# hbaatz/nerf-tex

Hardware: AMD Instinct MI355X
Metric: ray-samples/sec (MLP+composite) at 800x800x64 (higher is better)
Workload: dtype f32; 1 GPU; carpet 800x800x64: 640000 all-hit rays x 64 samples per GPU (BASELINE configs[1]), ParamNerf n_parameters=[1, 6], seeded glorot weights, inputs resident in HBM, fused PE+MLP+composite; rays_per_gpu=640000, hit_rays_total=640000, samples_per_ray=64

## Files before the change

### nerf_tex_amd/csrc/ntx_train.hip

```cpp
#include "nerftex.h"

#include <hip/hip_runtime.h>

#include <algorithm>
#include <cmath>
#include <cstdint>
#include <cstdio>
#include <cstdlib>
#include <cstring>
#include <type_traits>
#include <vector>

#include "ntx_train_device.h"

extern "C" int ntx_set_error(int code, const char *fmt, ...);

#define TRAIN_TRY(expr)                                                                                  \
    do {                                                                                                 \
        hipError_t e_ = (expr);                                                                          \
        if (e_ != hipSuccess) return ntx_set_error(NTX_E_HIP, "%s: %s", #expr, hipGetErrorString(e_)); \
    } while (0)

namespace ntx_train {

constexpr int TM = 128;

struct GemmArgs {
    const float *A; int lda; const float *B; int ldb; float *C; int ldc;
    int M, N, K;
    const float *bias;
    const float *mask; int ldmask;
    int relu, accumulate;
    int k_chunk; long long split_stride;
    float *colsum;
    int aligned;
};

template <int n, bool FAST>
__device__ __forceinline__ void fetch_run(const float *g, bool row_ok, int first, int bound, float *r, bool aligned_ok = false) {
    if (FAST) {
        const f32x4 *v = reinterpret_cast<const f32x4 *>(g);
#pragma unroll
        for (int q = 0; q < n / 4; ++q) { const f32x4 x = v[q]; r[4 * q] = x.x; r[4 * q + 1] = x.y; r[4 * q + 2] = x.z; r[4 * q + 3] = x.w; }
    } else if (row_ok && first + n <= bound && aligned_ok) {
        const f32x4 *v = reinterpret_cast<const f32x4 *>(g);
#pragma unroll
        for (int q = 0; q < n / 4; ++q) { const f32x4 x = v[q]; r[4 * q] = x.x; r[4 * q + 1] = x.y; r[4 * q + 2] = x.z; r[4 * q + 3] = x.w; }
    } else {
#pragma unroll
        for (int q = 0; q < n; ++q) r[q] = (row_ok && first + q < bound) ? g[q] : 0.0f;
    }
}

template <bool A_KCONTIG, int TN_, int TK_>
__device__ __forceinline__ void gemm_body(const GemmArgs &g, int bx, int by, int bz) {
    constexpr int THREADS = TN_ * 2, WCOLS = TN_ / 64, LROWA = TM + 4, LROWB_ = TN_ + 4;
    constexpr int FA = TM * TK_ / THREADS;
    constexpr int FB = TN_ * TK_ / THREADS;
    constexpr int TPR = THREADS / TK_;
    static_assert(FA % 4 == 0 && FB % 4 == 0 && FA * (THREADS / TM) == TK_ && TPR * FB == TN_ && TPR * FA == TM, "panel split");
    __shared__ __attribute__((aligned(16))) float As[2][TK_][LROWA], Bs[2][TK_][LROWB_];
    const int lane = threadIdx.x & 63, wave = threadIdx.x >> 6;
    const int j0 = bx * TN_, i0 = by * TM;
    const int k_begin = bz * g.k_chunk;
    const int k_end = k_begin + g.k_chunk < g.K ? k_begin + g.k_chunk : g.K;
    float *C = g.C + (size_t)bz * (size_t)g.split_stride;
    f32x16 acc[2][2];
#pragma unroll
    for (int a = 0; a < 2; ++a)
#pragma unroll
        for (int b = 0; b < 2; ++b)
#pragma unroll
            for (int r = 0; r < 16; ++r) acc[a][b][r] = 0.0f;
    float ra[2][FA], rb[2][FB], cs[FB];
#pragma unroll
    for (int q = 0; q < FB; ++q) cs[q] = 0.0f;
    const bool want_colsum = !A_KCONTIG && g.colsum != nullptr && by == 0;
    const bool inner = g.aligned && i0 + TM <= g.M && j0 + TN_ <= g.N;
    const int a_row = A_KCONTIG ? (int)(threadIdx.x % TM) : (int)(threadIdx.x / TPR), a_off = A_KCONTIG ? (int)(threadIdx.x / TM) * FA : (int)(threadIdx.x % TPR) * FA;
    const int b_row = (int)(threadIdx.x / TPR), b_off = (int)(threadIdx.x % TPR) * FB;
    auto fetch = [&](int k0, float *fa, float *fb) {
        const bool al = g.aligned != 0;
        if (A_KCONTIG) fetch_run<FA, false>(g.A + (size_t)(i0 + a_row) * g.lda + k0 + a_off, i0 + a_row < g.M, k0 + a_off, k_end, fa, al);
        else fetch_run<FA, false>(g.A + (size_t)(k0 + a_row) * g.lda + i0 + a_off, k0 + a_row < k_end, i0 + a_off, g.M, fa, al);
        fetch_run<FB, false>(g.B + (size_t)(k0 + b_row) * g.ldb + j0 + b_off, k0 + b_row < k_end, j0 + b_off, g.N, fb, al);
    };
    auto stash = [&](int buf, const float *fa, const float *fb) {
        if (want_colsum) {
#pragma unroll
            for (int q = 0; q < FB; ++q) cs[q] += fb[q];
        }
        if (A_KCONTIG) {
#pragma unroll
            for (int q = 0; q < FA; ++q) As[buf][a_off + q][a_row] = fa[q];
        } else {
            f32x4 *d = reinterpret_cast<f32x4 *>(&As[buf][a_row][a_off]);
#pragma unroll
            for (int q = 0; q < FA / 4; ++q) d[q] = f32x4{fa[4 * q], fa[4 * q + 1], fa[4 * q + 2], fa[4 * q + 3]};
        }
        f32x4 *d = reinterpret_cast<f32x4 *>(&Bs[buf][b_row][b_off]);
#pragma unroll
        for (int q = 0; q < FB / 4; ++q) d[q] = f32x4{fb[4 * q], fb[4 * q + 1], fb[4 * q + 2], fb[4 * q + 3]};
    };
    const int n_panels = (k_end - k_begin + TK_ - 1) / TK_;
    const int n_full = inner ? (k_end - k_begin) / TK_ : 0;
    const int wi = (wave / WCOLS) * 64 + 2 * (lane & 31), wj = (wave % WCOLS) * 64 + 2 * (lane & 31), kh = lane >> 5;
    const bool wave_live = j0 + (wave % WCOLS) * 64 < g.N;
    auto compute = [&](int buf) {
        if (!wave_live) return;
        f32x2 av[2], bv[2];
        av[0] = *reinterpret_cast<const f32x2 *>(&As[buf][kh][wi]); bv[0] = *reinterpret_cast<const f32x2 *>(&Bs[buf][kh][wj]);
#pragma unroll
        for (int st = 0; st < TK_ / 2; ++st) {
            const int c = st & 1, n = c ^ 1;
            if (st + 1 < TK_ / 2) {
                const int kk = 2 * (st + 1) + kh;
                av[n] = *reinterpret_cast<const f32x2 *>(&As[buf][kk][wi]); bv[n] = *reinterpret_cast<const f32x2 *>(&Bs[buf][kk][wj]);
            }
            __builtin_amdgcn_sched_barrier(0);
            acc[0][0] = __builtin_amdgcn_mfma_f32_32x32x2f32(av[c].x, bv[c].x, acc[0][0], 0, 0, 0);
            acc[0][1] = __builtin_amdgcn_mfma_f32_32x32x2f32(av[c].x, bv[c].y, acc[0][1], 0, 0, 0);
            acc[1][0] = __builtin_amdgcn_mfma_f32_32x32x2f32(av[c].y, bv[c].x, acc[1][0], 0, 0, 0);
            acc[1][1] = __builtin_amdgcn_mfma_f32_32x32x2f32(av[c].y, bv[c].y, acc[1][1], 0, 0, 0);
            __builtin_amdgcn_sched_barrier(0);
        }
    };
    auto fetch_fast = [&](int k0, float *fa, float *fb) {
        const float *ga = A_KCONTIG ? g.A + (size_t)(i0 + a_row) * g.lda + k0 + a_off : g.A + (size_t)(k0 + a_row) * g.lda + i0 + a_off;
        fetch_run<FA, true>(ga, true, 0, 0, fa);
        fetch_run<FB, true>(g.B + (size_t)(k0 + b_row) * g.ldb + j0 + b_off, true, 0, 0, fb);
    };
    auto pipeline = [&](auto fast_tag, int first, int last) {
        constexpr bool FAST = decltype(fast_tag)::value;
        auto get = [&](int kt, float *fa, float *fb) { if (FAST) fetch_fast(k_begin + kt * TK_, fa, fb); else fetch(k_begin + kt * TK_, fa, fb); };
        if (first >= last) return;
        get(first, ra[0], rb[0]); stash(0, ra[0], rb[0]);
        if (first + 1 < last) get(first + 1, ra[1], rb[1]);
        __syncthreads();
        int kt = first;
        for (; kt + 3 < last; kt += 2) {
            get(kt + 2, ra[0], rb[0]); compute(0); stash(1, ra[1], rb[1]); __syncthreads();
            get(kt + 3, ra[1], rb[1]); compute(1); stash(0, ra[0], rb[0]); __syncthreads();
        }
        for (; kt < last; ++kt) {
            const int buf = (kt - first) & 1;
            if (kt + 2 < last) { if (buf) get(kt + 2, ra[1], rb[1]); else get(kt + 2, ra[0], rb[0]); }
            compute(buf);
            if (kt + 1 < last) { if (buf) stash(0, ra[0], rb[0]); else stash(1, ra[1], rb[1]); }
            __syncthreads();
        }
    };
    pipeline(std::true_type{}, 0, n_full);
    pipeline(std::false_type{}, n_full, n_panels);
    const bool whole = i0 + TM <= g.M && j0 + TN_ <= g.N && (g.ldc % 2 == 0) && (!g.mask || g.ldmask % 2 == 0) && ((uintptr_t)C % 8 == 0) && ((uintptr_t)g.mask % 8 == 0);
    const int j = j0 + (wave % WCOLS) * 64 + 2 * (lane & 31);
    const float bj0 = (g.bias && j < g.N) ? g.bias[j] : 0.0f, bj1 = (g.bias && j + 1 < g.N) ? g.bias[j + 1] : 0.0f;
#pragma unroll
    for (int a = 0; a < 2; ++a)
#pragma unroll
        for (int r = 0; r < 16; ++r) {
            const int i = i0 + (wave / WCOLS) * 64 + 2 * (8 * (r >> 2) + (r & 3) + 4 * kh) + a;
            float v0 = acc[a][0][r], v1 = acc[a][1][r];
            float *c = C + (size_t)i * g.ldc + j;
            if (whole) {
                f32x2 *c2 = reinterpret_cast<f32x2 *>(c);
                if (g.accumulate) { const f32x2 o = *c2; v0 += o.x; v1 += o.y; }
                v0 += bj0; v1 += bj1;
                if (g.relu) { v0 = v0 > 0.0f ? v0 : 0.0f; v1 = v1 > 0.0f ? v1 : 0.0f; }
                if (g.mask) { const f32x2 mk = *reinterpret_cast<const f32x2 *>(g.mask + (size_t)i * g.ldmask + j); if (!(mk.x > 0.0f)) v0 = 0.0f; if (!(mk.y > 0.0f)) v1 = 0.0f; }
                *c2 = f32x2{v0, v1};
            } else if (i < g.M) {
#pragma unroll
                for (int b = 0; b < 2; ++b) {
                    if (j + b >= g.N) continue;
                    float v = b ? v1 : v0;
                    if (g.accumulate) v = v + c[b];
                    v = v + (b ? bj1 : bj0);
                    if (g.relu) v = v > 0.0f ? v : 0.0f;
                    if (g.mask && !(g.mask[(size_t)i * g.ldmask + j + b] > 0.0f)) v = 0.0f;
                    c[b] = v;
                }
            }
        }
    if (want_colsum) {
        float (*red)[LROWB_] = Bs[0];
#pragma unroll
        for (int q = 0; q < FB; ++q) red[b_row][b_off + q] = cs[q];
        __syncthreads();
        if ((int)threadIdx.x < TN_ && j0 + (int)threadIdx.x < g.N) {
            float sum = 0.0f;
            for (int q = 0; q < TK_; ++q) sum += red[q][threadIdx.x];
            g.colsum[(size_t)bz * g.N + j0 + threadIdx.x] = sum;
        }
    }
}


__device__ __forceinline__ void gemm_place(int lin, int nx, int ny, int nz, int &bx, int &by, int &bz) {
    const int tiles = nx * ny;
    if (nz % 8 == 0) {
        const int xcd = lin & 7, slot = lin >> 3, tile = slot % tiles;
        bz = (slot / tiles) * 8 + xcd; bx = tile % nx; by = tile / nx;
    } else { bx = lin % nx; by = (lin / nx) % ny; bz = lin / tiles; }
}
template <bool A_KCONTIG, int TN_, int TK_, int WAVES_PER_EU = 2>
__global__ __launch_bounds__(TN_ * 2) __attribute__((amdgpu_waves_per_eu(WAVES_PER_EU, 8))) void gemm_kernel(GemmArgs g) {
    int bx, by, bz;
    gemm_place(blockIdx.x + gridDim.x * (blockIdx.y + gridDim.y * blockIdx.z), gridDim.x, gridDim.y, gridDim.z, bx, by, bz);
    gemm_body<A_KCONTIG, TN_, TK_>(g, bx, by, bz);
}

constexpr int MAX_REDUCE_BATCH = 32;
struct ReduceJob { const float *partial; int n_split; long long stride, count, pair; float *out; long long first; };
struct ReduceBatch { ReduceJob job[MAX_REDUCE_BATCH]; int n; };
__global__ void reduce_batch_kernel(ReduceBatch b) {
    const long long g = (long long)blockIdx.x * blockDim.x + threadIdx.x;
    int j = 0;
    while (j + 1 < b.n && g >= b.job[j + 1].first) ++j;
    const ReduceJob &r = b.job[j];
    const long long e = g - r.first;
    if (e >= r.count) return;
    float s4[4] = {0.0f, 0.0f, 0.0f, 0.0f};
    auto at = [&](int z) { const float *p = r.partial + (size_t)z * r.stride + e; return r.pair > 0 ? p[0] + p[r.pair] : p[0]; };
    int z = 0;
    for (; z + 4 <= r.n_split; z += 4) {
#pragma unroll
        for (int q = 0; q < 4; ++q) s4[q] += at(z + q);
    }
    for (int q = 0; z < r.n_split; ++z, ++q) s4[q] += at(z);
    r.out[e] = (s4[0] + s4[1]) + (s4[2] + s4[3]);
}

enum { PACK_HIDDEN = 0, PACK_LINEAR = 1, PACK_AUX_ROW = 2, PACK_AUX_RGB = 3, PACK_COPY = 4 };
struct PackSeg {
    const float *src; long long sk, sc;
    int mode;
    int K, ncols, nt;
    float *dst; long long first, count;
};
struct PackArgs { const PackSeg *seg; int n_seg; long long total; };
__global__ void pack_kernel(PackArgs a) {
    const long long e = (long long)blockIdx.x * blockDim.x + threadIdx.x;
    if (e >= a.total) return;
    int lo = 0, hi = a.n_seg - 1;
    while (lo < hi) { const int mid = (lo + hi + 1) >> 1; if (a.seg[mid].first <= e) lo = mid; else hi = mid - 1; }
    const PackSeg &p = a.seg[lo];
    const long long o = e - p.first;
    float v = 0.0f;
    if (p.mode == PACK_COPY) v = p.src[o];
    else if (p.mode == PACK_AUX_ROW) {
        const int h = (int)(o >> 7) & 1, V = (int)(o & 127), k = hidden_row(V, h);
        v = k < p.K ? p.src[k * p.sk] : 0.0f;
    } else if (p.mode == PACK_AUX_RGB) {
        const int c = (int)(o >> 7), h = (int)(o >> 6) & 1, V = (int)(o & 63);
        v = p.src[hidden_row(V, h) * 3 + c];
    } else {
        const int c = (int)(o & 3), lane = (int)((o >> 2) & 63);
        const long long rec = o >> 8;
        const int G = p.nt / 4, g = (int)(rec % G), s = (int)(rec / G);
        const int f = lane & 31, kh = lane >> 5;
        const int k = p.mode == PACK_HIDDEN ? hidden_row(s, kh) : 2 * s + kh, col = 32 * (4 * g + c) + f;
        if (k < p.K && col < p.ncols) v = p.src[k * p.sk + col * p.sc];
    }
    p.dst[o] = v;
}

struct EncodeArgs {
    const float *rays_o, *rays_d, *z, *params, *cone;
    long long rays_per_param_row, M;
    int n_rays, S, n_geo, n_app, pos_freq, dir_freq, param_freq, blur_idx;
    float *posO; int ptiles;
    float *dirO; int dtiles;
    float *dists;
};
__global__ __launch_bounds__(64) void encode_kernel(EncodeArgs a) {
    const int lane = threadIdx.x, n = lane & 31, h = lane >> 5, blk = blockIdx.x, part = blockIdx.y;
    const long long m = (long long)blk * 32 + n;
    const bool valid = m < a.M;
    const int ray = valid ? (int)(m / a.S) : 0, s = valid ? (int)(m - (long long)ray * a.S) : 0;
    const float d[3] = {a.rays_d[3 * ray], a.rays_d[3 * ray + 1], a.rays_d[3 * ray + 2]};
    const float dn = sqrtf((d[0] * d[0] + d[1] * d[1]) + d[2] * d[2]);
    const float zr = a.z[(size_t)ray * a.S + s];
    const bool hit = isfinite(zr);
    const float z = hit ? zr : 0.0f;
    const int P = a.n_geo + a.n_app;
    const float *pr = a.params + (size_t)(ray / a.rays_per_param_row) * (P > 0 ? P : 1);
    auto param = [&](int c) { return c == a.blur_idx ? (hit ? pr[c] * (a.cone[ray] * z) : 0.0f) : pr[c]; };
    float *O = part == 0 ? a.posO : a.dirO;
    const int tiles = part == 0 ? a.ptiles : a.dtiles;
    auto put = [&](int row, float v) {
        if (!valid) v = 0.0f;
        O[(((size_t)blk * tiles + (row >> 5)) * 4 + (n >> 3)) * 256 + ((row & 31) + 32 * ((n >> 2) & 1)) * 4 + (n & 3)] = v;
    };
    auto fourier = [&](int r0, int D, int L, auto x) {
        if (h == 0) for (int c = 0; c < D; ++c) put(r0 + c, x(c));
        for (int f = 0; f < L; ++f)
            for (int c = 0; c < D; ++c) put(r0 + D + 2 * D * f + h * D + c, ntx::sin_q(ldexpf(1.0f, f) * x(c), h));
    };
    if (part == 0) {
        const float o[3] = {a.rays_o[3 * ray], a.rays_o[3 * ray + 1], a.rays_o[3 * ray + 2]};
        fourier(0, 3, a.pos_freq, [&](int c) { return o[c] + d[c] * z; });
        if (a.n_geo > 0) fourier(3 * (1 + 2 * a.pos_freq), a.n_geo, a.param_freq, [&](int c) { return param(c); });
    } else {
        fourier(0, 3, a.dir_freq, [&](int c) { return d[c] / dn; });
        if (a.n_app > 0) fourier(3 * (1 + 2 * a.dir_freq), a.n_app, a.param_freq, [&](int c) { return param(a.n_geo + c); });
        if (valid && h == 0) {
            const float zn = s + 1 < a.S ? a.z[(size_t)ray * a.S + s + 1] : 0.0f;
            const float dist = s + 1 < a.S ? zn - z : (a.S > 1 ? z - a.z[(size_t)ray * a.S + s - 1] : 0.0f);
            a.dists[(size_t)ray * a.S + s] = hit ? dist * dn : 0.0f;
        }
    }
}

__global__ __launch_bounds__(64) void encode_ipe_kernel(EncodeArgs a) {
    const int lane = threadIdx.x, n = lane & 31, h = lane >> 5, blk = blockIdx.x, part = blockIdx.y;
    const long long m = (long long)blk * 32 + n;
    const bool valid = m < a.M;
    const int ray = valid ? (int)(m / a.S) : 0, s = valid ? (int)(m - (long long)ray * a.S) : 0;
    const float d[3] = {a.rays_d[3 * ray], a.rays_d[3 * ray + 1], a.rays_d[3 * ray + 2]};
    const float dn = sqrtf((d[0] * d[0] + d[1] * d[1]) + d[2] * d[2]);
    const float *zr = a.z + (size_t)ray * (a.S + 1) + s;
    const float e0 = zr[0], e1 = zr[1];
    const bool hit = isfinite(e0) && isfinite(e1);
    const int P = a.n_geo + a.n_app;
    const float *pr = a.params + (size_t)(ray / a.rays_per_param_row) * (P + 1);
    auto param = [&](int k) { return pr[k < a.blur_idx ? k : k + 1]; };
    float *O = part == 0 ? a.posO : a.dirO;
    const int tiles = part == 0 ? a.ptiles : a.dtiles;
    auto put = [&](int row, float v) {
        if (!valid) v = 0.0f;
        O[(((size_t)blk * tiles + (row >> 5)) * 4 + (n >> 3)) * 256 + ((row & 31) + 32 * ((n >> 2) & 1)) * 4 + (n & 3)] = v;
    };
    auto fourier = [&](int r0, int D, int L, auto x) {
        if (h == 0) for (int c = 0; c < D; ++c) put(r0 + c, x(c));
        for (int f = 0; f < L; ++f)
            for (int c = 0; c < D; ++c) put(r0 + D + 2 * D * f + h * D + c, ntx::sin_q(ldexpf(1.0f, f) * x(c), h));
    };
    if (part == 0) {
        float mean[3] = {a.rays_o[3 * ray], a.rays_o[3 * ray + 1], a.rays_o[3 * ray + 2]}, cov[3] = {0.0f, 0.0f, 0.0f};
        if (hit) {
            float t_mean, t_var, r_var;
            ntx::cone_moments((e0 + e1) / 2.0f, (e1 - e0) / 2.0f, pr[a.blur_idx] * a.cone[ray], t_mean, t_var, r_var);
            for (int c = 0; c < 3; ++c) mean[c] = mean[c] + d[c] * t_mean;
            ntx::cone_cov(t_var, r_var, d, cov);
        }
        const int L = a.pos_freq;
        for (int f = 0; f < L; ++f)
            for (int c = 0; c < 3; ++c)
                put(h * 3 * L + 3 * f + c, ntx::sin_q(mean[c] * ldexpf(1.0f, f), h) * expf(-0.5f * (cov[c] * ldexpf(1.0f, 2 * f))));
        if (a.n_geo > 0) fourier(6 * L, a.n_geo, a.param_freq, [&](int c) { return param(c); });
    } else {
        fourier(0, 3, a.dir_freq, [&](int c) { return d[c] / dn; });
        if (a.n_app > 0) fourier(3 * (1 + 2 * a.dir_freq), a.n_app, a.param_freq, [&](int c) { return param(a.n_geo + c); });
        if (valid && h == 0) a.dists[(size_t)ray * a.S + s] = hit ? (e1 - e0) * dn : 0.0f;
    }
}

struct DirRowArgs {
    const float *rays_d, *params; long long rays_per_param_row;
    int n_rays, n_geo, n_app, dir_freq, param_freq, Kd, splice;
    const float *w, *bias;
    float *rows;
};
__global__ __launch_bounds__(256) void dirrow_kernel(DirRowArgs a) {
    __shared__ float feat[8 * MAX_PB_GROUPS];
    const int ray = blockIdx.x, f = threadIdx.x;
    const float d[3] = {a.rays_d[3 * ray], a.rays_d[3 * ray + 1], a.rays_d[3 * ray + 2]};
    const float dn = sqrtf((d[0] * d[0] + d[1] * d[1]) + d[2] * d[2]);
    const int P = a.n_geo + a.n_app + (a.splice >= 0 ? 1 : 0);
    const float *pr = a.params + (size_t)(ray / a.rays_per_param_row) * (P > 0 ? P : 1);
    if (f < a.Kd) {
        const int K3 = 3 * (1 + 2 * a.dir_freq);
        const int r = f < K3 ? f : f - K3, D = f < K3 ? 3 : a.n_app;
        auto x = [&](int c) { const int k = a.n_geo + c; return f < K3 ? d[c] / dn : pr[a.splice >= 0 && k >= a.splice ? k + 1 : k]; };
        float v;
        if (r < D) v = x(r);
        else { const int q = r - D, band = q / (2 * D), hc = q - band * 2 * D, hh = hc / D, c = hc - hh * D; v = ntx::sin_q(ldexpf(1.0f, band) * x(c), hh); }
        feat[f] = v;
    }
    __syncthreads();
    float acc = a.bias[f];
    for (int k = 0; k < a.Kd; ++k) acc = fmaf(feat[k], a.w[(size_t)k * 256 + f], acc);
    const int T = f >> 5, g = (f >> 3) & 3, h = (f >> 2) & 1, c = f & 3;
    a.rows[(size_t)ray * 256 + h * 128 + 16 * T + 4 * g + c] = acc;
}

struct CompositeArgs {
    const float *raw_rgb, *sigma, *dists;
    const float *noise;
    int n_rays, S, map_exr, composite_bkgd; float bkgd[3];
    const float *color_true, *alpha_true;
    int kind, loss_fn, alpha_loss_fn, filter_color_loss, use_hard_mask; float gamma;
    float *color, *alpha, *ray_loss;
    float *weights;
    float *dgrad;
    float *dhead;
    long long M;
};
constexpr int MAX_TRAIN_SAMPLES = 1024;
__device__ __forceinline__ float wave_sumf(float v) { for (int o = 32; o > 0; o >>= 1) v += __shfl_xor(v, o); return v; }
__device__ __forceinline__ float rgb_of(float raw, int map_exr) {
    if (map_exr) return raw > 0.0f ? raw + 1.0f : expf(raw);
    return 1.0f / (1.0f + expf(-raw));
}
__device__ __forceinline__ void loss_term(int fn, float t, float p, float inv_n, float &value, float &grad) {
    if (fn == NTX_LOSS_MSE) { const float e = t - p; value = e * e * inv_n; grad = -2.0f * e * inv_n; }
    else {
        const float e = t - p, den = (t + p) + 1e-2f, ae = fabsf(e);
        const float sgn = e > 0.0f ? 1.0f : (e < 0.0f ? -1.0f : 0.0f);
        value = ae / den * inv_n; grad = (-sgn / den - ae / (den * den)) * inv_n;
    }
}
__device__ __forceinline__ size_t dhead_at(long long m, int row) {
    const long long blk = m >> 5; const int p = (int)(m & 31);
    return (size_t)((blk * 4 + (p >> 3)) * 256 + (row + 32 * ((p >> 2) & 1)) * 4 + (p & 3));
}
__global__ __launch_bounds__(256) void composite_loss_kernel(CompositeArgs a) {
    __shared__ float sh_a[4][MAX_TRAIN_SAMPLES], sh_T[4][MAX_TRAIN_SAMPLES];
    const int lane = threadIdx.x & 63, wave = threadIdx.x >> 6;
    if (blockIdx.x == 0) {
        const long long end = (a.M + 31) / 32 * 32;
        for (long long m = a.M + threadIdx.x; m < end; m += 256)
            for (int r = 0; r < 4; ++r) a.dhead[dhead_at(m, r)] = 0.0f;
    }
    const int ray = blockIdx.x * 4 + wave;
    if (ray >= a.n_rays) return;
    const int S = a.S;
    const float *sg = a.sigma + (size_t)ray * S, *ds = a.dists + (size_t)ray * S, *rr = a.raw_rgb + (size_t)ray * S * 3;
    const float *nz = a.noise ? a.noise + (size_t)ray * S : nullptr;
    float *el = sh_a[wave], *T = sh_T[wave];
    for (int s = lane; s < S; s += 64) { const float v = nz ? sg[s] + nz[s] : sg[s]; const float r = v > 0.0f ? v : 0.0f; el[s] = expf(-r * ds[s]); }
    __builtin_amdgcn_wave_barrier();
    float carry = 1.0f;
    for (int s0 = 0; s0 < S; s0 += 64) {
        const int s = s0 + lane;
        float f = s < S ? el[s] + 1e-10f : 1.0f, incl = f;
        for (int o = 1; o < 64; o <<= 1) { const float w = __shfl_up(incl, o); if (lane >= o) incl *= w; }
        float excl = __shfl_up(incl, 1);
        if (lane == 0) excl = 1.0f;
        if (s < S) T[s] = carry * excl;
        carry *= __shfl(incl, 63);
    }
    __builtin_amdgcn_wave_barrier();
    float c0 = 0.0f, c1 = 0.0f, c2 = 0.0f, A = 0.0f;
    for (int s = lane; s < S; s += 64) {
        const float w = (1.0f - el[s]) * T[s];
        c0 += w * rgb_of(rr[3 * s], a.map_exr); c1 += w * rgb_of(rr[3 * s + 1], a.map_exr); c2 += w * rgb_of(rr[3 * s + 2], a.map_exr);
        A += w;
        if (a.weights) a.weights[(size_t)ray * S + s] = w;
    }
    c0 = wave_sumf(c0); c1 = wave_sumf(c1); c2 = wave_sumf(c2); A = wave_sumf(A);
    if (a.composite_bkgd) { c0 += (1.0f - A) * a.bkgd[0]; c1 += (1.0f - A) * a.bkgd[1]; c2 += (1.0f - A) * a.bkgd[2]; }
    const float cp[3] = {c0, c1, c2};
    float dC[3], dA = 0.0f, total = 0.0f;
    {
        const float inv_c = 1.0f / (float)(a.n_rays * 3), inv_a = 1.0f / (float)a.n_rays;
        float mask = 1.0f;
        if (a.kind == NTX_LOSS_ALPHA && a.filter_color_loss) mask = a.use_hard_mask ? (a.alpha_true[ray] > 0.0f ? 1.0f : 0.0f) : a.alpha_true[ray];
        for (int c = 0; c < 3; ++c) {
            float v, gr;
            loss_term(a.loss_fn, a.color_true[3 * ray + c] * mask, cp[c] * mask, inv_c, v, gr);
            total += v; dC[c] = gr * mask;
        }
        if (a.kind == NTX_LOSS_ALPHA) { float v; loss_term(a.alpha_loss_fn, a.alpha_true[ray], A, inv_a, v, dA); total += a.gamma * v; dA *= a.gamma; }
    }
    if (lane == 0) { a.color[3 * ray] = c0; a.color[3 * ray + 1] = c1; a.color[3 * ray + 2] = c2; a.alpha[ray] = A; a.ray_loss[ray] = total; }
    if (a.composite_bkgd) dA -= (dC[0] * a.bkgd[0] + dC[1] * a.bkgd[1]) + dC[2] * a.bkgd[2];
    float Z_carry = 1.0f, V_carry = 0.0f;
    for (int s0 = ((S - 1) / 64) * 64; s0 >= 0; s0 -= 64) {
        const int s = s0 + lane;
        float cs = 0.0f, rgb[3] = {0.0f, 0.0f, 0.0f}, e = 1.0f;
        float F = 1.0f, Bz = 0.0f, Bv = 0.0f;
        if (s < S) {
            e = el[s];
            for (int c = 0; c < 3; ++c) rgb[c] = rgb_of(rr[3 * s + c], a.map_exr);
            cs = (dC[0] * rgb[0] + dC[1] * rgb[1]) + dC[2] * rgb[2];
            F = e + 1e-10f; Bz = -1e-10f; Bv = cs * (1.0f - e);
        }
        for (int o = 1; o < 64; o <<= 1) {
            const float Fo = __shfl_down(F, o), Bzo = __shfl_down(Bz, o), Bvo = __shfl_down(Bv, o);
            if (lane + o < 64) { Bz = fmaf(F, Bzo, Bz); Bv = fmaf(F, Bvo, Bv); F *= Fo; }
        }
        float Fn = __shfl_down(F, 1), Bzn = __shfl_down(Bz, 1), Bvn = __shfl_down(Bv, 1);
        if (lane == 63) { Fn = 1.0f; Bzn = 0.0f; Bvn = 0.0f; }
        const float Z = fmaf(Fn, Z_carry, Bzn), V = fmaf(Fn, V_carry, Bvn);
        if (s < S) {
            const float w = (1.0f - e) * T[s];
            const float d_a = T[s] * fmaf(dA, Z, cs - V);
            const float sig = nz ? sg[s] + nz[s] : sg[s];
            float gr[4];
            for (int c = 0; c < 3; ++c) {
                const float raw = rr[3 * s + c];
                const float drgb = a.map_exr ? (raw > 0.0f ? 1.0f : expf(raw)) : rgb[c] * (1.0f - rgb[c]);
                gr[c] = w * dC[c] * drgb;
            }
            gr[3] = sig > 0.0f ? d_a * ds[s] * e : 0.0f;
            const long long m = (long long)ray * S + s;
            *reinterpret_cast<f32x4 *>(a.dgrad + 4 * m) = f32x4{gr[0], gr[1], gr[2], gr[3]};
            for (int r = 0; r < 4; ++r) a.dhead[dhead_at(m, r)] = gr[r];
        }
        const float F0 = __shfl(F, 0);
        Z_carry = fmaf(F0, Z_carry, __shfl(Bz, 0)); V_carry = fmaf(F0, V_carry, __shfl(Bv, 0));
    }
}
__global__ __launch_bounds__(1024) void loss_sum_kernel(const float *__restrict__ ray_loss, int n_rays, float *__restrict__ loss) {
    __shared__ float red[1024];
    float total = 0.0f;
    for (int r = threadIdx.x; r < n_rays; r += blockDim.x) total += ray_loss[r];
    red[threadIdx.x] = total;
    __syncthreads();
    for (int o = blockDim.x / 2; o > 0; o >>= 1) { if ((int)threadIdx.x < o) red[threadIdx.x] += red[threadIdx.x + o]; __syncthreads(); }
    if (threadIdx.x == 0) *loss = red[0];
}

__global__ void adam_kernel(float *__restrict__ w, const float *__restrict__ g, float *__restrict__ m, float *__restrict__ v, long long n, float lr_t, float b1,
                            float b2, float eps) {
    const long long e = (long long)blockIdx.x * blockDim.x + threadIdx.x;
    if (e >= n) return;
    const float ge = g[e];
    const float me = m[e] + (ge - m[e]) * (1.0f - b1);
    const float ve = v[e] + (ge * ge - v[e]) * (1.0f - b2);
    m[e] = me; v[e] = ve;
    w[e] = w[e] - (me * lr_t) / (sqrtf(ve) + eps);
}

}

struct TLayer { int in, out; size_t w, b; };

struct ntx_trainer {
    int device = 0, cus = 256;
    ntx_model_desc desc{};
    int Kp = 0, Kd = 0, P = 0, ptiles = 0, dtiles = 0, PS = 0, DS = 0;
    bool ipe = false;
    TLayer trunk[8], feature, c1, c2, rgb, alpha;
    size_t n_weights = 0;
    long long cap = 0, cap_blocks = 0, cap_rays = 0;
    float *w = nullptr, *grad = nullptr, *adam_m = nullptr, *adam_v = nullptr;
    float *wfwd = nullptr, *wdx = nullptr, *aux = nullptr; size_t fwd_floats = 0, dx_floats = 0;
    ntx_train::PackSeg *pack_seg = nullptr; int n_pack = 0; long long pack_total = 0;
    float *posO = nullptr, *dirO = nullptr;
    float *act = nullptr; long long act_stride = 0;
    unsigned int *bits = nullptr; long long bits_stride = 0;
    int fwd_variant = 0;
    float *sigma = nullptr, *raw_rgb = nullptr, *z = nullptr, *dists = nullptr, *noise = nullptr;
    float *dirrow = nullptr;
    float *dgrad = nullptr, *dhead = nullptr, *gout = nullptr; long long gout_stride = 0;
    ntx_train::DwJob *jobs = nullptr; int n_jobs = 0; long long total_cost = 0;
    std::vector<ntx_train::DwJob> jobs_host; std::vector<int> reduce_job;
    float *dw_partial = nullptr;
    ntx_train::ReduceBatch reduce{};
    float *color = nullptr, *alpha_out = nullptr, *ray_loss = nullptr, *loss = nullptr;
    float *weights_out = nullptr;
    float *stash = nullptr;
    long long adam_iterations = 0;
};

namespace {

using namespace ntx_train;


void free_all(ntx_trainer *t) {
    if (!t) return;
    (void)hipSetDevice(t->device);
    void *ptrs[] = {t->w, t->grad, t->adam_m, t->adam_v, t->wfwd, t->wdx, t->aux, t->pack_seg, t->posO, t->dirO, t->sigma, t->raw_rgb, t->z, t->dists, t->noise,
                    t->dgrad, t->dhead, t->jobs, t->dw_partial, t->stash, t->dirrow, t->color, t->alpha_out, t->ray_loss, t->loss, t->act, t->bits, t->gout};
    for (void *p : ptrs) if (p) (void)hipFree(p);
    delete t;
}

template <bool AK>
void launch_gemm(hipStream_t st, GemmArgs g) {
    g.k_chunk = g.K;
    g.aligned = (g.lda % 4 == 0) && (g.ldb % 4 == 0) && (((uintptr_t)g.A | (uintptr_t)g.B) % 16 == 0);
    hipLaunchKernelGGL((gemm_kernel<AK, 128, 16>), dim3((g.N + 127) / 128, (g.M + TM - 1) / TM, 1), dim3(256), 0, st, g);
}

}

namespace ntx_train {
template <int K, bool HOIST> void launch_fwd_variant(hipStream_t st, unsigned grid, const FwdArgs &a);
void launch_fwd_chain(int variant, bool hoist, hipStream_t st, unsigned grid, const FwdArgs &a) {
    switch (variant * 2 + (hoist ? 1 : 0)) {
        case 0: launch_fwd_variant<0, false>(st, grid, a); break;
        case 1: launch_fwd_variant<0, true>(st, grid, a); break;
        case 2: launch_fwd_variant<1, false>(st, grid, a); break;
        case 3: launch_fwd_variant<1, true>(st, grid, a); break;
        case 4: launch_fwd_variant<2, false>(st, grid, a); break;
        case 5: launch_fwd_variant<2, true>(st, grid, a); break;
        case 6: launch_fwd_variant<3, false>(st, grid, a); break;
        default: launch_fwd_variant<3, true>(st, grid, a); break;
    }
}
}

extern "C" {

int ntx_sample_depths(const float *t, int64_t n_rays, int n_points, uint32_t flags, uint64_t perturb_seed, const ntx_render_opts *opts, float *z_out,
                      ntx_stream stream);
int ntx_sample_noise(int64_t n_rays, int n_points, uint64_t seed, const ntx_render_opts *opts, float *noise_out, ntx_stream stream);

int ntx_trainer_create(const ntx_model_desc *desc, const float *weights, size_t n_floats, int device, int64_t max_rays, int max_samples_per_ray, ntx_trainer **out) {
    if (!out) return ntx_set_error(NTX_E_INVALID, "out is NULL");
    *out = nullptr;
    if (!desc || !weights) return ntx_set_error(NTX_E_INVALID, "desc / weights is NULL");
    const bool ipe = desc->pos_encoding == NTX_POS_IPE && desc->n_pos == 6;
    if (desc->kind != NTX_MODEL_PARAMNERF || desc->depth != 8 || desc->width != 256 || desc->skip != 4 || desc->color_depth != 1 ||
        !((desc->pos_encoding == NTX_POS_FOURIER && desc->n_pos == 3) || ipe))
        return ntx_set_error(NTX_E_UNSUPPORTED, "training is built for the ParamNerf architecture of the shipped training configs (depth 8, width 256, skips [4], color_depth 1, "
                                                "Fourier features on n_pos 3 or IPE on n_pos 6); others render but do not train");
    if (desc->n_geo < 0 || desc->n_app < 0 || desc->n_geo + desc->n_app > 16) return ntx_set_error(NTX_E_INVALID, "n_parameters out of range");
    if (desc->pos_freq < 0 || desc->dir_freq < 0 || desc->param_freq < 0) return ntx_set_error(NTX_E_INVALID, "negative band count");
    const int Kp = (ipe ? 6 * desc->pos_freq : 3 * (1 + 2 * desc->pos_freq)) + desc->n_geo * (1 + 2 * desc->param_freq), Kd = 3 * (1 + 2 * desc->dir_freq) + desc->n_app * (1 + 2 * desc->param_freq);
    if (Kp > 8 * MAX_PB_GROUPS || Kd > 8 * MAX_PB_GROUPS)
        return ntx_set_error(NTX_E_UNSUPPORTED, "training: pos_map (%d) / dir_map (%d) wider than %d features (the chain holds a block's encoded inputs in registers)", Kp, Kd,
                             8 * MAX_PB_GROUPS);
    if (max_rays < 1 || max_samples_per_ray < 2 || max_samples_per_ray > MAX_TRAIN_SAMPLES || max_rays * (int64_t)max_samples_per_ray > (int64_t)1 << 30)
        return ntx_set_error(NTX_E_INVALID, "max_rays / max_samples_per_ray out of range (samples per ray <= %d)", MAX_TRAIN_SAMPLES);
    int ndev = 0;
    if (hipGetDeviceCount(&ndev) != hipSuccess || ndev <= 0) return ntx_set_error(NTX_E_NODEVICE, "no HIP device visible");
    if (device < 0 || device >= ndev) return ntx_set_error(NTX_E_INVALID, "device %d out of range [0,%d)", device, ndev);
    ntx_trainer *t = new ntx_trainer();
    t->device = device; t->desc = *desc; t->ipe = ipe;
    t->P = desc->n_geo + desc->n_app; t->Kp = Kp; t->Kd = Kd;
    t->ptiles = (Kp + 31) / 32; t->dtiles = (Kd + 31) / 32;
    {
        const int psg = ((Kp + 1) / 2 + 3) / 4, dsg = ((Kd + 1) / 2 + 3) / 4;
        t->fwd_variant = 3;
        for (int v = 2; v >= 0; --v)
            if (FWD_VARIANTS[v][0] >= psg && FWD_VARIANTS[v][1] >= dsg &&
                FWD_VARIANTS[v][0] + FWD_VARIANTS[v][1] <= FWD_VARIANTS[t->fwd_variant][0] + FWD_VARIANTS[t->fwd_variant][1]) t->fwd_variant = v;
        t->PS = 4 * FWD_VARIANTS[t->fwd_variant][0]; t->DS = 4 * FWD_VARIANTS[t->fwd_variant][1];
    }
    size_t p = 0;
    auto take = [&](int in, int o) { TLayer l{in, o, p, p + (size_t)in * o}; p += (size_t)in * o + o; return l; };
    int k = Kp;
    for (int i = 0; i < 8; ++i) { t->trunk[i] = take(k, 256); k = 256 + (i == 4 ? Kp : 0); }
    t->feature = take(256, 256); t->c1 = take(256 + Kd, 256); t->c2 = take(256, 128); t->rgb = take(128, 3); t->alpha = take(256, 1);
    t->n_weights = p;
    if (n_floats != p) { delete t; return ntx_set_error(NTX_E_INVALID, "weights: %zu floats, the model has %zu", n_floats, p); }
    const long long M = (long long)max_rays * max_samples_per_ray, NB = (M + 31) / 32;
    t->cap = M; t->cap_rays = max_rays; t->cap_blocks = NB;
    int rc = hipSetDevice(device) == hipSuccess ? NTX_OK : ntx_set_error(NTX_E_HIP, "hipSetDevice(%d) failed", device);
    if (rc == NTX_OK) { int n = 0; if (hipDeviceGetAttribute(&n, hipDeviceAttributeMultiprocessorCount, device) == hipSuccess && n > 0) t->cus = n; }
    auto alloc = [&](float **d, size_t n, bool zero = false) -> int {
        if (rc != NTX_OK) return rc;
        if (hipMalloc((void **)d, (n ? n : 1) * sizeof(float)) != hipSuccess) return rc = ntx_set_error(NTX_E_HIP, "hipMalloc of %zu floats failed", n);
        if (zero && hipMemset(*d, 0, (n ? n : 1) * sizeof(float)) != hipSuccess) return rc = ntx_set_error(NTX_E_HIP, "hipMemset failed");
        return rc;
    };
    alloc(&t->w, p); alloc(&t->grad, p, true); alloc(&t->adam_m, p, true); alloc(&t->adam_v, p, true);
    alloc(&t->posO, (size_t)NB * t->ptiles * 1024, true); alloc(&t->dirO, (size_t)NB * t->dtiles * 1024, true);
    t->act_stride = t->gout_stride = NB * 8 * 1024; t->bits_stride = NB * 256;
    alloc(&t->act, (size_t)t->act_stride * 11); alloc((float **)&t->bits, (size_t)t->bits_stride * 10); alloc(&t->gout, (size_t)t->gout_stride * 11);
    auto act = [&](int i) { return t->act + (size_t)i * t->act_stride; };
    auto gout = [&](int i) { return t->gout + (size_t)i * t->gout_stride; };
    alloc(&t->sigma, (size_t)M); alloc(&t->raw_rgb, (size_t)M * 3); alloc(&t->z, (size_t)(M + max_rays)); alloc(&t->dists, (size_t)M); alloc(&t->noise, (size_t)M);
    alloc(&t->dirrow, (size_t)max_rays * 256);
    alloc(&t->dgrad, (size_t)NB * 32 * 4); alloc(&t->dhead, (size_t)NB * 1024, true);
    alloc(&t->color, (size_t)max_rays * 3); alloc(&t->alpha_out, (size_t)max_rays); alloc(&t->ray_loss, (size_t)max_rays); alloc(&t->loss, 1);
    if (rc == NTX_OK && hipMemcpy(t->w, weights, p * sizeof(float), hipMemcpyHostToDevice) != hipSuccess) rc = ntx_set_error(NTX_E_HIP, "weight upload failed");
    std::vector<PackSeg> segs;
    long long first = 0;
    auto seg = [&](const float *src, long long sk, long long sc, int mode, int K, int ncols, int nt, size_t *stream_floats, int nsteps) {
        PackSeg s{}; s.src = src; s.sk = sk; s.sc = sc; s.mode = mode; s.K = K; s.ncols = ncols; s.nt = nt;
        const int ring = stream_floats == &t->dx_floats ? DX_RING : RING;
        const long long recs = ((long long)nsteps * (nt / 4) + ring - 1) / ring * ring;
        s.count = recs * 256; s.first = first; s.dst = (float *)(uintptr_t)(*stream_floats * sizeof(float));
        first += s.count; *stream_floats += (size_t)s.count;
        segs.push_back(s);
    };
    const float *W = t->w;
    auto fwd_hidden = [&](const TLayer &l, int row0, int nt) { seg(W + l.w + (size_t)row0 * l.out, l.out, 1, PACK_HIDDEN, 256, l.out, nt, &t->fwd_floats, 128); };
    auto fwd_linear = [&](const TLayer &l, int K, int nsteps) { seg(W + l.w, l.out, 1, PACK_LINEAR, K, l.out, 8, &t->fwd_floats, nsteps); };
    fwd_linear(t->trunk[0], Kp, t->PS);
    for (int i = 1; i < 8; ++i) {
        if (i == 5) { fwd_linear(t->trunk[5], Kp, t->PS); fwd_hidden(t->trunk[5], Kp, 8); }
        else fwd_hidden(t->trunk[i], 0, 8);
    }
    fwd_hidden(t->feature, 0, 8);
    fwd_linear(t->c1, Kd, t->DS); fwd_hidden(t->c1, Kd, 8);
    fwd_hidden(t->c2, 0, 4);
    const size_t n_fwd_segs = segs.size();
    auto dx_hidden = [&](const TLayer &l, int row0, int K, int nsteps) { seg(W + l.w + (size_t)row0 * l.out, 1, l.out, PACK_HIDDEN, K, 256, 8, &t->dx_floats, nsteps); };
    seg(W + t->rgb.w, 1, 3, PACK_LINEAR, 3, 128, 4, &t->dx_floats, 2);
    dx_hidden(t->c2, 0, 128, 64);
    dx_hidden(t->c1, Kd, 256, 128);
    dx_hidden(t->feature, 0, 256, 128);
    seg(W + t->alpha.w, 1, 1, PACK_LINEAR, 1, 256, 8, &t->dx_floats, 1);
    for (int i = 7; i >= 1; --i) dx_hidden(t->trunk[i], i == 5 ? Kp : 0, 256, 128);
    const size_t n_stream_segs = segs.size();
    auto tail = [&](size_t of, size_t *stream_floats) { PackSeg s = segs[of]; s.count = (long long)(stream_floats == &t->dx_floats ? DX_RING : RING) * 256; s.first = first; s.dst = (float *)(uintptr_t)(*stream_floats * sizeof(float));
                                                        first += s.count; *stream_floats += (size_t)s.count; segs.push_back(s); };
    tail(0, &t->fwd_floats); tail(n_fwd_segs, &t->dx_floats);
    auto aux_seg = [&](const float *src, int mode, int K, long long count, size_t at) {
        PackSeg s{}; s.src = src; s.sk = 1; s.mode = mode; s.K = K; s.count = count; s.first = first; s.dst = (float *)(uintptr_t)(at * sizeof(float));
        first += count; segs.push_back(s);
    };
    for (int i = 0; i < 8; ++i) aux_seg(W + t->trunk[i].b, PACK_AUX_ROW, 256, 256, AUX_BIAS + (size_t)i * 256);
    aux_seg(W + t->feature.b, PACK_AUX_ROW, 256, 256, AUX_BIAS + 8 * 256); aux_seg(W + t->c1.b, PACK_AUX_ROW, 256, 256, AUX_BIAS + 9 * 256);
    aux_seg(W + t->c2.b, PACK_AUX_ROW, 128, 256, AUX_BIAS + 10 * 256);
    aux_seg(W + t->alpha.w, PACK_AUX_ROW, 256, 256, AUX_ALPHA_W); aux_seg(W + t->alpha.b, PACK_COPY, 1, 1, AUX_ALPHA_B);
    aux_seg(W + t->rgb.w, PACK_AUX_RGB, 128, 384, AUX_RGB_W); aux_seg(W + t->rgb.b, PACK_COPY, 3, 3, AUX_RGB_B);
    t->pack_total = first; t->n_pack = (int)segs.size();
    alloc(&t->wfwd, t->fwd_floats); alloc(&t->wdx, t->dx_floats); alloc(&t->aux, AUX_FLOATS, true);
    if (rc == NTX_OK) {
        for (size_t i = 0; i < segs.size(); ++i) {
            const bool is_aux = i >= n_stream_segs + 2, is_fwd = i < n_fwd_segs || i == n_stream_segs;
            float *base = is_aux ? t->aux : is_fwd ? t->wfwd : t->wdx;
            segs[i].dst = (float *)((char *)base + (uintptr_t)segs[i].dst);
        }
        if (hipMalloc((void **)&t->pack_seg, segs.size() * sizeof(PackSeg)) != hipSuccess ||
            hipMemcpy(t->pack_seg, segs.data(), segs.size() * sizeof(PackSeg), hipMemcpyHostToDevice) != hipSuccess)
            rc = ntx_set_error(NTX_E_HIP, "segment table upload failed");
    }
    std::vector<DwJob> &jobs = t->jobs_host;
    struct RJ { int job; long long at, count, pair; size_t out; };
    std::vector<RJ> rjobs;
    auto new_job = [&]() { DwJob j{}; for (DwWave &w : j.w) w.shape = -1; jobs.push_back(j); return (int)jobs.size() - 1; };
    auto matrix = [&](int j, int K, int N, size_t g_kernel, long long g_bias, long long *at_bias) {
        const long long at = jobs[j].slot_floats;
        jobs[j].slot_floats += (long long)K * N;
        rjobs.push_back(RJ{j, at, (long long)K * N, 0, g_kernel});
        *at_bias = -1;
        if (g_bias >= 0) { *at_bias = jobs[j].slot_floats; jobs[j].slot_floats += 2 * N; rjobs.push_back(RJ{j, *at_bias, N, N, (size_t)g_bias}); }
        return at;
    };
    auto wave = [&](int j, int w, int shape, const float *A, int rtA, int a0, const float *B, int rtB, int b0, long long at, int K, int N, int c_lo, long long at_bias) {
        DwWave &d = jobs[j].w[w];
        d.A = A; d.rtA = rtA; d.a0 = a0; d.B = B; d.rtB = rtB; d.b0 = b0; d.shape = shape; d.out = at; d.ldc = N; d.row0 = a0 * 32; d.rows_valid = K;
        d.col0 = b0 * 32; d.c_lo = c_lo; d.c_hi = c_lo + N; d.bias_out = a0 == 0 ? at_bias : -1;
        const int cost = shape == 0 ? 256 : shape == 1 ? 198 : 68;
        if (cost > jobs[j].cost) jobs[j].cost = cost;
    };
    auto layer_job = [&](const float *X, const float *dY, size_t g_kernel, size_t g_bias) {
        const int j = new_job(); long long ab; const long long at = matrix(j, 256, 256, g_kernel, (long long)g_bias, &ab);
        for (int w = 0; w < 4; ++w) wave(j, w, 0, X, 8, 4 * (w >> 1), dY, 8, 4 * (w & 1), at, 256, 256, 0, ab);
    };
    {
        const TLayer &r = t->rgb, &al = t->alpha, &c2 = t->c2, &c1 = t->c1, &f = t->feature;
        for (int i = 7; i >= 1; --i) layer_job(act(i - 1), gout(10 - i), t->trunk[i].w + (size_t)(i == 5 ? Kp : 0) * 256, t->trunk[i].b);
        layer_job(act(7), gout(2), f.w, f.b);
        layer_job(act(8), gout(1), c1.w + (size_t)Kd * 256, c1.b);
        {
            const int j = new_job(); long long ab0, ab5;
            const long long at0 = matrix(j, Kp, 256, t->trunk[0].w, (long long)t->trunk[0].b, &ab0), at5 = matrix(j, Kp, 256, t->trunk[5].w, -1, &ab5);
            for (int w = 0; w < 2; ++w) { wave(j, w, 1, t->posO, t->ptiles, 0, gout(10), 8, 4 * w, at0, Kp, 256, 0, ab0); wave(j, 2 + w, 1, t->posO, t->ptiles, 0, gout(5), 8, 4 * w, at5, Kp, 256, 0, ab5); }
        }
        {
            const int j = new_job(); long long abd, ab2;
            const long long atd = matrix(j, Kd, 256, c1.w, -1, &abd), at2 = matrix(j, 256, 128, c2.w, (long long)c2.b, &ab2);
            for (int w = 0; w < 2; ++w) { wave(j, w, 1, t->dirO, t->dtiles, 0, gout(1), 8, 4 * w, atd, Kd, 256, 0, abd); wave(j, 2 + w, 0, act(9), 8, 4 * w, gout(0), 4, 0, at2, 256, 128, 0, ab2); }
        }
        {
            const int j = new_job(); long long abr, aba;
            const long long atr = matrix(j, 128, 3, r.w, (long long)r.b, &abr), ata = matrix(j, 256, 1, al.w, (long long)al.b, &aba);
            wave(j, 0, 2, act(10), 4, 0, t->dhead, 1, 0, atr, 128, 3, 0, abr);
            for (int w = 0; w < 2; ++w) wave(j, 1 + w, 2, act(7), 8, 4 * w, t->dhead, 1, 0, ata, 256, 1, 3, aba);
        }
    }
    t->n_jobs = (int)jobs.size();
    size_t partial_floats = 0;
    for (DwJob &j : jobs) {
        t->total_cost += j.cost;
    }
    for (DwJob &j : jobs) {
        const long long slots = ((long long)j.cost * t->cus + t->total_cost - 1) / t->total_cost + 2;
        j.first_float = (long long)partial_floats; partial_floats += (size_t)(slots * j.slot_floats);
    }
    alloc(&t->dw_partial, partial_floats);
    if (rc == NTX_OK) {
        if (hipMalloc((void **)&t->jobs, jobs.size() * sizeof(DwJob)) != hipSuccess ||
            hipMemcpy(t->jobs, jobs.data(), jobs.size() * sizeof(DwJob), hipMemcpyHostToDevice) != hipSuccess)
            rc = ntx_set_error(NTX_E_HIP, "job table upload failed");
        if ((int)rjobs.size() > MAX_REDUCE_BATCH) rc = ntx_set_error(NTX_E_INVALID, "trainer: too many weight gradients for one launch");
        long long rfirst = 0;
        for (size_t i = 0; i < rjobs.size() && rc == NTX_OK; ++i) {
            ReduceJob &r = t->reduce.job[t->reduce.n++];
            const DwJob &j = jobs[rjobs[i].job];
            r.partial = t->dw_partial + j.first_float + rjobs[i].at; r.n_split = 0; r.stride = j.slot_floats; r.count = rjobs[i].count; r.pair = rjobs[i].pair;
            r.out = t->grad + rjobs[i].out; r.first = rfirst;
            rfirst += (rjobs[i].count + 255) / 256 * 256;
            t->reduce_job.push_back(rjobs[i].job);
        }
    }
    if (rc != NTX_OK) { free_all(t); return rc; }
    *out = t;
    return NTX_OK;
}

int ntx_trainer_destroy(ntx_trainer *t) { free_all(t); return NTX_OK; }

size_t ntx_trainer_weight_count(const ntx_trainer *t) { return t ? t->n_weights : 0; }

static float *trainer_vector(ntx_trainer *t, int what) {
    return what == NTX_TRAINER_WEIGHTS ? t->w : what == NTX_TRAINER_GRADIENTS ? t->grad : what == NTX_TRAINER_ADAM_M ? t->adam_m : what == NTX_TRAINER_ADAM_V ? t->adam_v : nullptr;
}

int ntx_trainer_get(ntx_trainer *t, int what, float *out_host, size_t n_floats) {
    if (!t || !out_host) return ntx_set_error(NTX_E_INVALID, "NULL argument");
    if (n_floats != t->n_weights) return ntx_set_error(NTX_E_INVALID, "%zu floats asked, the model has %zu", n_floats, t->n_weights);
    const float *src = trainer_vector(t, what);
    if (!src) return ntx_set_error(NTX_E_INVALID, "what = %d", what);
    TRAIN_TRY(hipSetDevice(t->device));
    TRAIN_TRY(hipDeviceSynchronize());
    TRAIN_TRY(hipMemcpy(out_host, src, n_floats * sizeof(float), hipMemcpyDeviceToHost));
    return NTX_OK;
}

int ntx_trainer_activation(ntx_trainer *t, int layer, int64_t n_samples_total, float *out_host) {
    if (!t || !out_host) return ntx_set_error(NTX_E_INVALID, "NULL argument");
    if (n_samples_total < 1 || n_samples_total > t->cap) return ntx_set_error(NTX_E_INVALID, "n_samples_total out of range");
    const float *src = nullptr; int tiles = 8;
    auto act = [&](int i) { return t->act + (size_t)i * t->act_stride; };
    auto gout = [&](int i) { return t->gout + (size_t)i * t->gout_stride; };
    if (layer >= 0 && layer < 8) src = act(layer);
    else if (layer == 8) src = act(9);
    else if (layer == 9) { src = act(10); tiles = 4; }
    else if (layer == 10) src = t->sigma;
    else if (layer >= 20 && layer < 28) src = gout(10 - (layer - 20));
    else if (layer == 28) src = gout(1);
    else if (layer == 29) src = gout(2);
    else if (layer == 11) src = t->raw_rgb;
    else if (layer == 30) src = t->dgrad;
    else return ntx_set_error(NTX_E_INVALID, "layer %d (0-7 trunk, 8 / 9 the colour layers, 10 the density, 11 the raw colour; 20-29 the kept gradients, 30 the composite's adjoint)", layer);
    TRAIN_TRY(hipSetDevice(t->device));
    TRAIN_TRY(hipDeviceSynchronize());
    if (layer == 10 || layer == 11 || layer == 30) {
        const size_t width = layer == 10 ? 1 : (layer == 11 ? 3 : 4);
        TRAIN_TRY(hipMemcpy(out_host, src, (size_t)n_samples_total * width * sizeof(float), hipMemcpyDeviceToHost)); return NTX_OK;
    }
    const long long nb = (n_samples_total + 31) / 32;
    std::vector<float> tmp((size_t)nb * tiles * 1024);
    TRAIN_TRY(hipMemcpy(tmp.data(), src, tmp.size() * sizeof(float), hipMemcpyDeviceToHost));
    const int width = tiles * 32;
    for (long long m = 0; m < n_samples_total; ++m) {
        const long long blk = m >> 5; const int p = (int)(m & 31);
        const float *rec = tmp.data() + ((size_t)blk * tiles * 4 + (p >> 3)) * 256 + 32 * ((p >> 2) & 1) * 4 + (p & 3);
        float *o = out_host + (size_t)m * width;
        for (int T = 0; T < tiles; ++T)
            for (int i = 0; i < 32; ++i) o[32 * T + i] = rec[(size_t)T * 1024 + i * 4];
    }
    return NTX_OK;
}

int ntx_trainer_set_weights(ntx_trainer *t, const float *weights_host, size_t n_floats) { return ntx_trainer_set(t, NTX_TRAINER_WEIGHTS, weights_host, n_floats); }

int ntx_trainer_set(ntx_trainer *t, int what, const float *values_host, size_t n_floats) {
    if (!t || !values_host) return ntx_set_error(NTX_E_INVALID, "NULL argument");
    if (n_floats != t->n_weights) return ntx_set_error(NTX_E_INVALID, "%zu floats given, the model has %zu", n_floats, t->n_weights);
    float *dst = trainer_vector(t, what);
    if (!dst) return ntx_set_error(NTX_E_INVALID, "what = %d", what);
    TRAIN_TRY(hipSetDevice(t->device));
    TRAIN_TRY(hipDeviceSynchronize());
    TRAIN_TRY(hipMemcpy(dst, values_host, n_floats * sizeof(float), hipMemcpyHostToDevice));
    return NTX_OK;
}

int ntx_trainer_set_iterations(ntx_trainer *t, int64_t iterations) {
    if (!t || iterations < 0) return ntx_set_error(NTX_E_INVALID, "trainer is NULL or iterations < 0");
    t->adam_iterations = iterations;
    return NTX_OK;
}

int ntx_trainer_composite_weights(ntx_trainer *t, float *weights_dev) {
    if (!t) return ntx_set_error(NTX_E_INVALID, "trainer is NULL");
    if (t->ipe && weights_dev) return ntx_set_error(NTX_E_UNSUPPORTED, "an IPE trainer has no importance pass (MipRenderer: renderer.py:403-404)");
    t->weights_out = weights_dev;
    return NTX_OK;
}

namespace ntx_train {
__global__ void add_kernel(float *__restrict__ dst, const float *__restrict__ src, long long n) {
    const long long e = (long long)blockIdx.x * blockDim.x + threadIdx.x;
    if (e < n) dst[e] += src[e];
}
}

int ntx_trainer_stash_gradients(ntx_trainer *t, int op, ntx_stream stream) {
    if (!t || (op != 0 && op != 1)) return ntx_set_error(NTX_E_INVALID, "trainer is NULL or op is not 0 (keep) / 1 (add back)");
    TRAIN_TRY(hipSetDevice(t->device));
    if (!t->stash) {
        if (op == 1) return ntx_set_error(NTX_E_INVALID, "no gradient was kept");
        TRAIN_TRY(hipMalloc((void **)&t->stash, t->n_weights * sizeof(float)));
    }
    if (op == 0) TRAIN_TRY(hipMemcpyAsync(t->stash, t->grad, t->n_weights * sizeof(float), hipMemcpyDeviceToDevice, (hipStream_t)stream));
    else hipLaunchKernelGGL(ntx_train::add_kernel, dim3((unsigned)((t->n_weights + 255) / 256)), dim3(256), 0, (hipStream_t)stream, t->grad, t->stash, (long long)t->n_weights);
    TRAIN_TRY(hipGetLastError());
    return NTX_OK;
}

int ntx_trainer_device_weights(ntx_trainer *t, const float **weights_dev) {
    if (!t || !weights_dev) return ntx_set_error(NTX_E_INVALID, "NULL argument");
    *weights_dev = t->w;
    return NTX_OK;
}

int ntx_trainer_allreduce_gradients(ntx_trainer *t, ntx_comm *comm, ntx_stream stream) {
    if (!t || !comm) return ntx_set_error(NTX_E_INVALID, "NULL argument");
    return ntx_allreduce_mean_f32(comm, t->grad, t->n_weights, stream);
}

int ntx_train_step_gradients(ntx_trainer *t, const float *rays_o, const float *rays_d, const float *tnear_far, const float *params, int64_t rays_per_param_row,
                             const float *cone_scale, int64_t n_rays, int n_samples, int blur_idx, uint32_t flags, const float *bkgd, uint64_t perturb_seed,
                             const ntx_render_opts *opts, const float *z_vals, const float *color_true, const float *alpha_true, const ntx_loss_desc *loss,
                             float *color_pred, float *alpha_pred, float *loss_out, ntx_stream stream) {
    if (!t) return ntx_set_error(NTX_E_INVALID, "trainer is NULL");
    const int P_in = t->P + (t->ipe ? 1 : 0);
    if (!rays_o || !rays_d || (!tnear_far && !z_vals) || !color_true || !loss || (P_in > 0 && !params)) return ntx_set_error(NTX_E_INVALID, "NULL buffer");
    if (n_rays < 1 || n_rays > t->cap_rays || n_samples < 2 || (long long)n_rays * n_samples > t->cap) return ntx_set_error(NTX_E_INVALID, "n_rays x n_samples beyond what the trainer was created for");
    if (n_samples > MAX_TRAIN_SAMPLES) return ntx_set_error(NTX_E_INVALID, "n_samples > %d", MAX_TRAIN_SAMPLES);
    if (blur_idx >= P_in || (blur_idx >= 0 && !cone_scale) || (t->ipe && blur_idx < 0)) return ntx_set_error(NTX_E_INVALID, "bad blur_idx / cone_scale");
    if (loss->size < sizeof(ntx_loss_desc) || (loss->kind != NTX_LOSS_NERF && loss->kind != NTX_LOSS_ALPHA) || (loss->loss_fn != NTX_LOSS_MSE && loss->loss_fn != NTX_LOSS_SMAPE) ||
        (loss->alpha_loss_fn != NTX_LOSS_MSE && loss->alpha_loss_fn != NTX_LOSS_SMAPE))
        return ntx_set_error(NTX_E_INVALID, "bad ntx_loss_desc");
    if (loss->kind == NTX_LOSS_ALPHA && !alpha_true) return ntx_set_error(NTX_E_INVALID, "AlphaLoss needs alpha_true");
    if (rays_per_param_row < 1) rays_per_param_row = 1;
    TRAIN_TRY(hipSetDevice(t->device));
    hipStream_t st = (hipStream_t)stream;
    const long long M = (long long)n_rays * n_samples;
    const int S = n_samples, n_blocks = (int)((M + 31) / 32);
    {
        PackArgs pa{t->pack_seg, t->n_pack, t->pack_total};
        hipLaunchKernelGGL(pack_kernel, dim3((unsigned)((t->pack_total + 255) / 256)), dim3(256), 0, st, pa);
    }
    const float *z = z_vals;
    if (!z) {
        int rc = ntx_sample_depths(tnear_far, n_rays, t->ipe ? S + 1 : S, flags & NTX_FLAG_PERTURB, perturb_seed, opts, t->z, stream);
        if (rc != NTX_OK) return rc;
        z = t->z;
    }
    const float *noise = nullptr;
    if (flags & NTX_FLAG_RAW_NOISE) {
        int rc = ntx_sample_noise(n_rays, S, perturb_seed, opts, t->noise, stream);
        if (rc != NTX_OK) return rc;
        noise = t->noise;
    }
    {
        EncodeArgs e{}; e.rays_o = rays_o; e.rays_d = rays_d; e.z = z; e.params = params; e.cone = cone_scale; e.rays_per_param_row = rays_per_param_row; e.M = M;
        e.n_rays = (int)n_rays; e.S = S; e.n_geo = t->desc.n_geo; e.n_app = t->desc.n_app; e.pos_freq = t->desc.pos_freq; e.dir_freq = t->desc.dir_freq;
        e.param_freq = t->desc.param_freq; e.blur_idx = blur_idx; e.posO = t->posO; e.ptiles = t->ptiles; e.dirO = t->dirO;
        e.dtiles = t->dtiles; e.dists = t->dists;
        if (t->ipe) hipLaunchKernelGGL(encode_ipe_kernel, dim3((unsigned)n_blocks, 2), dim3(64), 0, st, e);
        else hipLaunchKernelGGL(encode_kernel, dim3((unsigned)n_blocks, 2), dim3(64), 0, st, e);
    }
    const unsigned chain_grid = (unsigned)std::min<long long>(t->cus, (n_blocks + 3) / 4);
    {
        FwdArgs f{}; f.stream = t->wfwd; f.stream_bytes = (uint32_t)(t->fwd_floats * sizeof(float)); f.aux = t->aux; f.M = M;
        f.ptiles = t->ptiles; f.dtiles = t->dtiles; f.pos = t->posO; f.dir = t->dirO;
        f.act = t->act; f.act_stride = t->act_stride; f.bits = t->bits; f.bits_stride = t->bits_stride;
        f.sigma = t->sigma; f.raw_rgb = t->raw_rgb;
        const bool hoist = (t->ipe || blur_idx < 0 || blur_idx < t->desc.n_geo) && S % 32 == 0 && getenv("NERFTEX_TRAIN_NO_DIR_HOIST") == nullptr;
        if (hoist) {
            DirRowArgs dr{}; dr.rays_d = rays_d; dr.params = params; dr.rays_per_param_row = rays_per_param_row; dr.n_rays = (int)n_rays; dr.n_geo = t->desc.n_geo;
            dr.n_app = t->desc.n_app; dr.dir_freq = t->desc.dir_freq; dr.param_freq = t->desc.param_freq; dr.Kd = t->Kd; dr.w = t->w + t->c1.w; dr.bias = t->w + t->c1.b;
            dr.rows = t->dirrow; dr.splice = t->ipe ? blur_idx : -1;
            hipLaunchKernelGGL(dirrow_kernel, dim3((unsigned)n_rays), dim3(256), 0, st, dr);
        }
        f.dirrow = t->dirrow; f.n_rays = (int)n_rays; f.S = S;
        launch_fwd_chain(t->fwd_variant, hoist, st, chain_grid, f);
    }
    {
        CompositeArgs c{};
        c.raw_rgb = t->raw_rgb; c.sigma = t->sigma; c.dists = t->dists; c.noise = noise; c.n_rays = (int)n_rays; c.S = S; c.map_exr = (flags & NTX_FLAG_MAP_EXR) ? 1 : 0;
        c.composite_bkgd = (flags & NTX_FLAG_COMPOSITE_BKGD) ? 1 : 0;
        for (int k = 0; k < 3; ++k) c.bkgd[k] = bkgd ? bkgd[k] : 1.0f;
        c.color_true = color_true; c.alpha_true = alpha_true; c.kind = loss->kind; c.loss_fn = loss->loss_fn; c.alpha_loss_fn = loss->alpha_loss_fn;
        c.filter_color_loss = loss->filter_color_loss; c.use_hard_mask = loss->use_hard_mask; c.gamma = loss->gamma;
        c.weights = t->weights_out;
        c.color = color_pred ? color_pred : t->color; c.alpha = alpha_pred ? alpha_pred : t->alpha_out; c.ray_loss = t->ray_loss; c.dgrad = t->dgrad; c.dhead = t->dhead; c.M = M;
        hipLaunchKernelGGL(composite_loss_kernel, dim3((unsigned)((n_rays + 3) / 4)), dim3(256), 0, st, c);
        hipLaunchKernelGGL(loss_sum_kernel, dim3(1), dim3(1024), 0, st, t->ray_loss, (int)n_rays, loss_out ? loss_out : t->loss);
    }
    {
        DxArgs d{}; d.stream = t->wdx; d.stream_bytes = (uint32_t)(t->dx_floats * sizeof(float)); d.M = M; d.dgrad = t->dgrad;
        d.out = t->gout; d.out_stride = t->gout_stride; d.bits = t->bits; d.bits_stride = t->bits_stride;
        launch_dx_chain(st, chain_grid, d);
    }
    {
        DwArgs d{}; d.jobs = t->jobs; d.n_jobs = t->n_jobs; d.n_blocks = n_blocks; d.total_cost = t->total_cost; d.partial = t->dw_partial;
        const long long G = t->cus, W = t->total_cost * n_blocks;
#ifdef NTX_TRAIN_CLOCKS
        static unsigned long long *clocks = nullptr;
        const size_t nck = (size_t)G * (2 + 3 * t->n_jobs);
        if (getenv("NERFTEX_DW_CLOCKS")) {
            if (!clocks) (void)hipMalloc((void **)&clocks, nck * sizeof(unsigned long long));
            (void)hipMemsetAsync(clocks, 0, nck * sizeof(unsigned long long), st);
            d.clocks = clocks;
        }
#endif
        launch_dw(st, (unsigned)G, d);
#ifdef NTX_TRAIN_CLOCKS
        if (d.clocks) {
            std::vector<unsigned long long> h(nck);
            (void)hipStreamSynchronize(st);
            (void)hipMemcpy(h.data(), clocks, nck * sizeof(unsigned long long), hipMemcpyDeviceToHost);
            unsigned long long t0 = ~0ull;
            for (long long g = 0; g < G; ++g) t0 = std::min(t0, h[g * (2 + 3 * t->n_jobs)]);
            FILE *f = fopen(getenv("NERFTEX_DW_CLOCKS"), "w");
            if (f) {
                for (long long g = 0; g < G; ++g) {
                    const unsigned long long *c = &h[g * (2 + 3 * t->n_jobs)];
                    fprintf(f, "%lld %llu %llu", g, c[0] - t0, c[1] - t0);
                    for (int j = 0; j < t->n_jobs; ++j) if (c[4 + 3 * j]) fprintf(f, "  j%d cost %d blocks %llu %llu-%llu", j, t->jobs_host[j].cost, c[2 + 3 * j], c[3 + 3 * j] - t0, c[4 + 3 * j] - t0);
                    fprintf(f, "\n");
                }
                fclose(f);
            }
        }
#endif
        ReduceBatch rb = t->reduce;
        std::vector<int> slots(t->n_jobs);
        long long start = 0;
        for (int j = 0; j < t->n_jobs; ++j) {
            const long long span = (long long)t->jobs_host[j].cost * n_blocks;
            slots[j] = (int)(dw_last_g(G, W, start, span) - dw_first_g(G, W, start) + 1);
            start += span;
        }
        for (int i = 0; i < rb.n; ++i) rb.job[i].n_split = slots[t->reduce_job[i]];
        const long long total = rb.job[rb.n - 1].first + (rb.job[rb.n - 1].count + 255) / 256 * 256;
        hipLaunchKernelGGL(reduce_batch_kernel, dim3((unsigned)(total / 256)), dim3(256), 0, st, rb);
    }
    TRAIN_TRY(hipGetLastError());
    return NTX_OK;
}

int ntx_trainer_adam_step(ntx_trainer *t, float lrate, float lrate_decay_steps, float lrate_decay_rate, float beta_1, float beta_2, float epsilon, ntx_stream stream) {
    if (!t) return ntx_set_error(NTX_E_INVALID, "trainer is NULL");
    TRAIN_TRY(hipSetDevice(t->device));
    const double step = (double)t->adam_iterations;
    double lr = lrate;
    if (lrate_decay_steps > 0) lr = (double)lrate * std::pow((double)lrate_decay_rate, step / (double)lrate_decay_steps);
    const double tt = step + 1.0;
    const float lr_t = (float)((double)(float)lr * std::sqrt(1.0 - std::pow((double)beta_2, tt)) / (1.0 - std::pow((double)beta_1, tt)));
    hipLaunchKernelGGL(ntx_train::adam_kernel, dim3((unsigned)((t->n_weights + 255) / 256)), dim3(256), 0, (hipStream_t)stream, t->w, t->grad, t->adam_m, t->adam_v,
                       (long long)t->n_weights, lr_t, beta_1, beta_2, epsilon);
    t->adam_iterations += 1;
    TRAIN_TRY(hipGetLastError());
    return NTX_OK;
}

int64_t ntx_trainer_iterations(const ntx_trainer *t) { return t ? t->adam_iterations : -1; }

int ntx_gemm_f32(const float *A, int lda, int a_kcontig, const float *B, int ldb, int b_kcontig, float *C, int ldc, int M, int N, int K, const float *bias, int relu,
                 ntx_stream stream) {
    if (!A || !B || !C || M < 1 || N < 1 || K < 1) return ntx_set_error(NTX_E_INVALID, "bad GEMM arguments");
    ntx_train::GemmArgs g{}; g.A = A; g.lda = lda; g.B = B; g.ldb = ldb; g.C = C; g.ldc = ldc; g.M = M; g.N = N; g.K = K; g.bias = bias; g.relu = relu;
    hipStream_t st = (hipStream_t)stream;
    if (b_kcontig) return ntx_set_error(NTX_E_UNSUPPORTED, "B must be [K][N]");
    if (a_kcontig) launch_gemm<true>(st, g); else launch_gemm<false>(st, g);
    TRAIN_TRY(hipGetLastError());
    return NTX_OK;
}

}
```

### nerf_tex_amd/csrc/ntx_train_device.h

```cpp
#pragma once

#include "ntx_device.h"

namespace ntx_train {

using ntx::f32x16;
using ntx::f32x4;
using ntx::hidden_row;
using ntx::mfma32;
using ntx::RING;
using ntx::static_for;
typedef float f32x2 __attribute__((ext_vector_type(2)));
typedef int i32x4 __attribute__((ext_vector_type(4)));
typedef unsigned int u32x4 __attribute__((ext_vector_type(4)));

#define TRN_DEV __device__ __forceinline__

TRN_DEV __amdgpu_buffer_rsrc_t make_rsrc(const void *base, long long bytes) {
    const long long b = bytes < 0 ? 0 : (bytes > 0x7ffffff0ll ? 0x7ffffff0ll : bytes);
    return __builtin_amdgcn_make_buffer_rsrc(const_cast<void *>(base), 0, (int)b, 0x00020000);
}

TRN_DEV uint32_t o_lane_bytes(int lane) {
    const int n = lane & 31, h = lane >> 5;
    return (uint32_t)((n >> 3) * 1024 + ((n >> 2) & 1) * 512 + h * 64 + (n & 3) * 4);
}
constexpr int STORE_NT = 0;
constexpr uint32_t o_value_bytes(int V) { return (uint32_t)((V >> 4) * 4096 + ((V & 15) >> 2) * 128 + (V & 3) * 16); }

template <int R>
struct WRingT {
    static constexpr int DEPTH = R;
    __amdgpu_buffer_rsrc_t rsrc;
    uint32_t voff;
    f32x4 r[R];
};
typedef WRingT<RING> WRing;
constexpr int DX_RING = 16;
template <class WR>
TRN_DEV f32x4 wr_load(const WR &w, uint32_t byte_off) {
#ifdef NTX_X_WSMALL
    byte_off &= 0xffffu;
#endif
#ifdef NTX_X_NOWLOAD
    if (byte_off >= (uint32_t)WR::DEPTH * 1024u) return w.r[(byte_off >> 10) % WR::DEPTH];
#endif
    return __builtin_bit_cast(f32x4, __builtin_amdgcn_raw_buffer_load_b128(w.rsrc, w.voff, byte_off, 0));
}

template <int NSTEPS, int NMT, bool ZERO, class WR, class Extra>
TRN_DEV void seg_hidden(f32x16 (&acc)[8], WR &ws, uint32_t &sbase, const float (&hin)[128], Extra &&extra) {
    constexpr int RPS = NMT / 4, RING = WR::DEPTH;
    static_assert((NSTEPS * RPS) % RING == 0, "whole ring turns");
    const f32x16 zero = {0.f, 0.f, 0.f, 0.f, 0.f, 0.f, 0.f, 0.f, 0.f, 0.f, 0.f, 0.f, 0.f, 0.f, 0.f, 0.f};
    static_for<NSTEPS>([&](auto S) {
        constexpr int s = S;
        f32x4 w;
        static_for<NMT>([&](auto MT) {
            constexpr int mt = MT;
            if constexpr (mt % 4 == 0) {
                constexpr int rec = s * RPS + mt / 4;
                w = ws.r[rec % RING];
                ws.r[rec % RING] = wr_load(ws, sbase + (uint32_t)(rec + RING) * 1024u);
            }
            if constexpr (ZERO && s == 0) acc[mt] = mfma32(w[mt % 4], hin[s], zero);
            else acc[mt] = mfma32(w[mt % 4], hin[s], acc[mt]);
            extra(S, MT);
            __builtin_amdgcn_sched_barrier(0);
        });
    });
    sbase += (uint32_t)(NSTEPS * RPS) * 1024u;
}

template <int NG, class Fetch>
TRN_DEV void seg_mem(f32x16 (&acc)[8], WRing &ws, uint32_t &sbase, float (&pb)[12], Fetch &&fetch) {
    static_assert(RING == 8, "a group of 4 k-steps of 8 tiles is one ring turn");
    static_for<NG>([&](auto G) {
        constexpr int g = G;
        if constexpr (g + 2 < NG) fetch(std::integral_constant<int, g + 2>{});
        static_for<4>([&](auto K) {
            constexpr int k = K;
            f32x4 w;
            static_for<8>([&](auto MT) {
                constexpr int mt = MT;
                if constexpr (mt % 4 == 0) {
                    constexpr int slot = 2 * k + mt / 4;
                    w = ws.r[slot];
                    ws.r[slot] = wr_load(ws, sbase + (uint32_t)(8 * g + slot + RING) * 1024u);
                }
                acc[mt] = mfma32(w[mt % 4], pb[4 * (g % 3) + k], acc[mt]);
                __builtin_amdgcn_sched_barrier(0);
            });
        });
    });
    sbase += (uint32_t)NG * 8192u;
}

template <int NKS, int NMT, bool ZERO, class WR>
TRN_DEV void seg_few(f32x16 (&acc)[8], WR &ws, uint32_t &sbase, const float (&b)[NKS]) {
    constexpr int RPS = NMT / 4, RING = WR::DEPTH;
    static_assert(NKS * RPS <= RING, "one ring turn");
    const f32x16 zero = {0.f, 0.f, 0.f, 0.f, 0.f, 0.f, 0.f, 0.f, 0.f, 0.f, 0.f, 0.f, 0.f, 0.f, 0.f, 0.f};
    static_for<RING>([&](auto I) {
        constexpr int rec = I;
        const f32x4 w = ws.r[rec];
        ws.r[rec] = wr_load(ws, sbase + (uint32_t)(rec + RING) * 1024u);
        if constexpr (rec < NKS * RPS) {
            constexpr int s = rec / RPS, t0 = 4 * (rec % RPS);
            static_for<4>([&](auto C) {
                constexpr int c = C;
                if constexpr (ZERO && s == 0) acc[t0 + c] = mfma32(w[c], b[s], zero);
                else acc[t0 + c] = mfma32(w[c], b[s], acc[t0 + c]);
                __builtin_amdgcn_sched_barrier(0);
            });
        }
    });
    sbase += (uint32_t)RING * 1024u;
}

template <int V0>
TRN_DEV void convert8_relu_bits(float (&hin)[128], const f32x16 (&prev)[8], uint32_t &w) {
    constexpr int T = V0 >> 4, R = V0 & 15;
    float t0, t1, t2, t3;
    asm("v_accvgpr_read_b32 %0, %13\n\tv_accvgpr_read_b32 %1, %14\n\tv_accvgpr_read_b32 %2, %15\n\tv_accvgpr_read_b32 %3, %16\n\t"
        "v_accvgpr_read_b32 %4, %17\n\tv_accvgpr_read_b32 %5, %18\n\tv_accvgpr_read_b32 %6, %19\n\tv_accvgpr_read_b32 %7, %20\n\t"
        "v_sub_f32 %9, 0, %0\n\tv_sub_f32 %10, 0, %1\n\tv_sub_f32 %11, 0, %2\n\tv_sub_f32 %12, 0, %3\n\t"
        "v_alignbit_b32 %8, %8, %9, 31\n\tv_alignbit_b32 %8, %8, %10, 31\n\tv_alignbit_b32 %8, %8, %11, 31\n\tv_alignbit_b32 %8, %8, %12, 31\n\t"
        "v_sub_f32 %9, 0, %4\n\tv_sub_f32 %10, 0, %5\n\tv_sub_f32 %11, 0, %6\n\tv_sub_f32 %12, 0, %7\n\t"
        "v_alignbit_b32 %8, %8, %9, 31\n\tv_alignbit_b32 %8, %8, %10, 31\n\tv_alignbit_b32 %8, %8, %11, 31\n\tv_alignbit_b32 %8, %8, %12, 31\n\t"
        "v_max_f32 %0, 0, %0\n\tv_max_f32 %1, 0, %1\n\tv_max_f32 %2, 0, %2\n\tv_max_f32 %3, 0, %3\n\t"
        "v_max_f32 %4, 0, %4\n\tv_max_f32 %5, 0, %5\n\tv_max_f32 %6, 0, %6\n\tv_max_f32 %7, 0, %7"
        : "=&v"(hin[V0 + 0]), "=&v"(hin[V0 + 1]), "=&v"(hin[V0 + 2]), "=&v"(hin[V0 + 3]), "=&v"(hin[V0 + 4]), "=&v"(hin[V0 + 5]), "=&v"(hin[V0 + 6]),
          "=&v"(hin[V0 + 7]), "+v"(w), "=&v"(t0), "=&v"(t1), "=&v"(t2), "=&v"(t3)
        : "a"(prev[T][R + 0]), "a"(prev[T][R + 1]), "a"(prev[T][R + 2]), "a"(prev[T][R + 3]), "a"(prev[T][R + 4]), "a"(prev[T][R + 5]), "a"(prev[T][R + 6]),
          "a"(prev[T][R + 7]));
}
constexpr int keep_bit(int V) { return 31 - (V & 31); }

template <int NMT>
TRN_DEV void convert_relu_bits(float (&hin)[128], const f32x16 (&prev)[8], u32x4 &bits) {
    static_for<(NMT + 1) / 2>([&](auto W) {
        constexpr int wd = W;
        uint32_t w = 0;
        static_for<(NMT - 2 * wd >= 2 ? 4 : 2)>([&](auto Q) { convert8_relu_bits<32 * wd + 8 * decltype(Q)::value>(hin, prev, w); });
        bits[wd] = w;
    });
}
template <int NMT>
TRN_DEV void convert_linear(float (&hin)[128], const f32x16 (&prev)[8]) {
    static_for<NMT * 16>([&](auto V) { constexpr int v = V; hin[v] = prev[v >> 4][v & 15]; });
}
template <int NMT>
TRN_DEV void convert_mask(float (&hin)[128], const f32x16 (&prev)[8], const u32x4 &bits) {
    static_for<NMT * 16>([&](auto V) {
        constexpr int v = V;
        const float x = prev[v >> 4][v & 15];
        const int keep = __builtin_amdgcn_sbfe((int)bits[v >> 5], keep_bit(v), 1);
        hin[v] = __builtin_bit_cast(float, __builtin_bit_cast(int, x) & keep);
    });
}

constexpr int AUX_BIAS = 0, AUX_ALPHA_W = 11 * 256, AUX_ALPHA_B = AUX_ALPHA_W + 256, AUX_RGB_W = AUX_ALPHA_B + 4, AUX_RGB_B = AUX_RGB_W + 384,
              AUX_FLOATS = AUX_RGB_B + 4;
template <int MT>
TRN_DEV void bias_tile(f32x16 (&acc)[8], const float *aux, int layer, int h) {
    const f32x4 *b = reinterpret_cast<const f32x4 *>(aux + AUX_BIAS + layer * 256 + h * 128) + MT * 4;
    const f32x4 v0 = b[0], v1 = b[1], v2 = b[2], v3 = b[3];
    acc[MT] = f32x16{v0.x, v0.y, v0.z, v0.w, v1.x, v1.y, v1.z, v1.w, v2.x, v2.y, v2.z, v2.w, v3.x, v3.y, v3.z, v3.w};
}

constexpr int MAX_PB_GROUPS = 12;
struct FwdArgs {
    const float *stream; uint32_t stream_bytes;
    const float *aux;
    long long M;
    int ptiles, dtiles;
    const float *pos, *dir;
    float *act; long long act_stride;
    unsigned int *bits; long long bits_stride;
    float *sigma, *raw_rgb;
    const float *dirrow; int n_rays, S;
};

#ifdef NTX_TRAIN_FWD
template <int PSG, int DSG, bool HOIST>
__global__ __launch_bounds__(256) __attribute__((amdgpu_waves_per_eu(1, 1))) void fwd_chain_kernel(FwdArgs a) {
    __shared__ __attribute__((aligned(16))) float aux_lds[AUX_FLOATS];
    __shared__ __attribute__((aligned(16))) float rows_lds[HOIST ? 4 * 256 : 4];
    ntx::load_aux(aux_lds, a.aux, AUX_FLOATS);
    const int lane = threadIdx.x & 63, n = lane & 31, h = lane >> 5;
    const int wave = __builtin_amdgcn_readfirstlane(blockIdx.x * 4 + (threadIdx.x >> 6)), nwaves = gridDim.x * 4;
    const int n_blocks = (int)((a.M + 31) >> 5);
    if (wave >= n_blocks) return;
    WRing ws;
    ws.rsrc = make_rsrc(a.stream, a.stream_bytes);
    ws.voff = (uint32_t)lane * 16u;
    static_for<RING>([&](auto I) { ws.r[I] = wr_load(ws, (uint32_t)decltype(I)::value * 1024u); });
    const uint32_t lane_o = o_lane_bytes(lane), lane_r = (uint32_t)((n >> 3) * 1024 + ((n >> 2) & 1) * 512 + (n & 3) * 4 + h * 16), lane16 = (uint32_t)lane * 16u;
    float pb[12];
    const __amdgpu_buffer_rsrc_t rs_row = make_rsrc(a.dirrow, HOIST ? (long long)a.n_rays * 1024 : 0);
    __amdgpu_buffer_rsrc_t rs_in = make_rsrc(a.pos + (size_t)wave * a.ptiles * 1024, (long long)a.ptiles * 4096);
    auto fetch = [&](auto G) {
        constexpr int g = G;
        static_for<4>([&](auto K) {
            constexpr int k = K;
            constexpr int s = 4 * g + k;
            pb[4 * (g % 3) + k] = __builtin_bit_cast(float, __builtin_amdgcn_raw_buffer_load_b32(rs_in, lane_r, (uint32_t)((s >> 4) * 4096 + (s & 15) * 32), 0));
        });
    };
    fetch(std::integral_constant<int, 0>{}); fetch(std::integral_constant<int, 1>{});
    for (int blk = wave; blk < n_blocks; blk += nwaves) {
        uint32_t opaque_zero = 0;
        asm volatile("" : "+v"(opaque_zero));
        const float *aux = aux_lds + opaque_zero;
        const float *rows_aux = rows_lds + opaque_zero + (HOIST ? (threadIdx.x >> 6) * 256 : 0) - AUX_BIAS - 9 * 256;
        uint32_t sbase = 0;
        f32x16 acc[8];
        float hin[128];
        const long long m = (long long)blk * 32 + n;
        const bool valid = m < a.M;
        if constexpr (HOIST) {
            const uint32_t ray = __builtin_amdgcn_readfirstlane((int)(((uint32_t)blk * 32u) / (uint32_t)a.S));
            const f32x4 x0 = __builtin_bit_cast(f32x4, __builtin_amdgcn_raw_buffer_load_b128(rs_row, lane16, (ray < (uint32_t)a.n_rays ? ray : (uint32_t)a.n_rays - 1u) * 1024u, 0));
            *reinterpret_cast<f32x4 *>(rows_lds + (threadIdx.x >> 6) * 256 + lane * 4) = x0;
            __builtin_amdgcn_wave_barrier();
        }
        __amdgpu_buffer_rsrc_t rs_out = make_rsrc(a.act, 0);
        auto leaves_to = [&](int idx, int tiles) { rs_out = make_rsrc(a.act + (size_t)idx * a.act_stride + (size_t)blk * tiles * 1024, (long long)tiles * 4096); };
        auto leave = [&](auto V) {
            constexpr int v = V;
#ifndef NTX_X_NOSTORE
            __builtin_amdgcn_raw_buffer_store_b32(__builtin_bit_cast(int, hin[v]), rs_out, lane_o, o_value_bytes(v), STORE_NT);
#endif
        };
        auto bits_leave = [&](int idx, const u32x4 &bw) {
#ifndef NTX_X_NOBITS
            const __amdgpu_buffer_rsrc_t rb = make_rsrc(a.bits + (size_t)idx * a.bits_stride + (size_t)blk * 256, 1024);
            __builtin_amdgcn_raw_buffer_store_b128(__builtin_bit_cast(i32x4, bw), rb, lane16, 0, 0);
#endif
        };
        static_for<8>([&](auto T) { bias_tile<decltype(T)::value>(acc, aux, 0, h); });
        seg_mem<PSG>(acc, ws, sbase, pb, fetch);
        float sig_part = 0.0f;
        auto layer = [&](auto LIc) {
            f32x16 (&cur)[8] = acc; f32x16 (&prev)[8] = acc;
            constexpr int LI = decltype(LIc)::value, in_idx = LI - 1;
            constexpr bool relu_in = in_idx != 8;
            u32x4 bw = {0u, 0u, 0u, 0u};
            if constexpr (HOIST && LI == 9) {
                sbase += (uint32_t)DSG * 8192u;
                static_for<RING>([&](auto I) { ws.r[I] = wr_load(ws, sbase + (uint32_t)decltype(I)::value * 1024u); });
            }
            static_for<4>([&](auto W) {
                constexpr int wd = W;
                if constexpr (relu_in) {
                    uint32_t w = 0;
                    static_for<4>([&](auto Q) { convert8_relu_bits<32 * wd + 8 * decltype(Q)::value>(hin, prev, w); });
                    bw[wd] = w;
                } else static_for<32>([&](auto V) { constexpr int v = 32 * wd + decltype(V)::value; hin[v] = prev[v >> 4][v & 15]; });
                const float *bsrc = (HOIST && LI == 9) ? rows_aux : aux;
                if constexpr (LI < 10 || wd < 2) { bias_tile<2 * wd>(cur, bsrc, LI, h); bias_tile<2 * wd + 1>(cur, bsrc, LI, h); }
            });
            if constexpr (relu_in) bits_leave(in_idx < 8 ? in_idx : 8, bw);
            if constexpr (LI == 8) {
                const f32x4 *wa = reinterpret_cast<const f32x4 *>(aux + AUX_ALPHA_W + h * 128);
                static_for<32>([&](auto I) {
                    constexpr int i = I;
                    const f32x4 w = wa[i];
                    sig_part = __builtin_fmaf(hin[4 * i + 0], w.x, sig_part); sig_part = __builtin_fmaf(hin[4 * i + 1], w.y, sig_part);
                    sig_part = __builtin_fmaf(hin[4 * i + 2], w.z, sig_part); sig_part = __builtin_fmaf(hin[4 * i + 3], w.w, sig_part);
                });
            }
            __builtin_amdgcn_sched_barrier(0);
            leaves_to(in_idx, 8);
            if constexpr (LI == 5) seg_mem<PSG>(cur, ws, sbase, pb, fetch);
            if constexpr (LI == 9 && !HOIST) seg_mem<DSG>(cur, ws, sbase, pb, fetch);
            if constexpr (LI == 4) rs_in = make_rsrc(a.pos + (size_t)blk * a.ptiles * 1024, (long long)a.ptiles * 4096);
            if constexpr (LI == 8 && !HOIST) rs_in = make_rsrc(a.dir + (size_t)blk * a.dtiles * 1024, (long long)a.dtiles * 4096);
            if constexpr (LI == 10) {
                const int nb = blk + nwaves < n_blocks ? blk + nwaves : blk;
                rs_in = make_rsrc(a.pos + (size_t)nb * a.ptiles * 1024, (long long)a.ptiles * 4096);
            }
            auto extra = [&](auto S, auto MT) {
                constexpr int s = decltype(S)::value, mt = decltype(MT)::value;
                if constexpr ((LI == 4 || (LI == 8 && !HOIST) || LI == 10) && mt == 2 && (s == 8 || s == 24)) fetch(std::integral_constant<int, (s == 8 ? 0 : 1)>{});
                if constexpr (mt == 5 || (LI == 10 && mt == 3)) leave(S);
            };
            if constexpr (LI == 10) seg_hidden<128, 4, false>(cur, ws, sbase, hin, extra);
            else seg_hidden<128, 8, false>(cur, ws, sbase, hin, extra);
        };
        static_for<10>([&](auto I) { layer(std::integral_constant<int, decltype(I)::value + 1>{}); });
        {
            u32x4 bw = {0u, 0u, 0u, 0u};
            convert_relu_bits<4>(hin, acc, bw);
            bits_leave(9, bw);
            leaves_to(10, 4);
            static_for<64>([&](auto V) { leave(V); });
            float rgb[3];
            static_for<3>([&](auto C) {
                constexpr int c = C;
                const f32x4 *wc = reinterpret_cast<const f32x4 *>(aux + AUX_RGB_W + (c * 2 + h) * 64);
                float p = 0.0f;
                static_for<16>([&](auto I) {
                    constexpr int i = I;
                    const f32x4 w = wc[i];
                    p = __builtin_fmaf(hin[4 * i + 0], w.x, p); p = __builtin_fmaf(hin[4 * i + 1], w.y, p);
                    p = __builtin_fmaf(hin[4 * i + 2], w.z, p); p = __builtin_fmaf(hin[4 * i + 3], w.w, p);
                });
                rgb[c] = p + __shfl_xor(p, 32, 64) + aux[AUX_RGB_B + c];
            });
            const float sigma = sig_part + __shfl_xor(sig_part, 32, 64) + aux[AUX_ALPHA_B];
            if (valid && h == 0) {
                a.sigma[m] = sigma;
                a.raw_rgb[3 * m + 0] = rgb[0]; a.raw_rgb[3 * m + 1] = rgb[1]; a.raw_rgb[3 * m + 2] = rgb[2];
            }
        }
    }
}

#endif

struct DxArgs {
    const float *stream; uint32_t stream_bytes;
    long long M;
    const float *dgrad;
    float *out; long long out_stride;
    const unsigned int *bits; long long bits_stride;
};

#ifdef NTX_TRAIN_DX
__global__ __launch_bounds__(256) __attribute__((amdgpu_waves_per_eu(1, 1))) void dx_chain_kernel(DxArgs a) {
    const int lane = threadIdx.x & 63, n = lane & 31, h = lane >> 5;
    const int wave = __builtin_amdgcn_readfirstlane(blockIdx.x * 4 + (threadIdx.x >> 6)), nwaves = gridDim.x * 4;
    const int n_blocks = (int)((a.M + 31) >> 5);
    if (wave >= n_blocks) return;
    WRingT<DX_RING> ws;
    ws.rsrc = make_rsrc(a.stream, a.stream_bytes);
    ws.voff = (uint32_t)lane * 16u;
    static_for<DX_RING>([&](auto I) { ws.r[I] = wr_load(ws, (uint32_t)decltype(I)::value * 1024u); });
    const uint32_t lane_o = o_lane_bytes(lane), lane16 = (uint32_t)lane * 16u;
    auto fetch_grad = [&](int blk) {
        const long long m = (long long)blk * 32 + n;
        const f32x4 zero = {0.0f, 0.0f, 0.0f, 0.0f};
        return m < a.M ? *reinterpret_cast<const f32x4 *>(a.dgrad + 4 * m) : zero;
    };
    f32x4 g = fetch_grad(wave);
    for (int blk = wave; blk < n_blocks; blk += nwaves) {
        uint32_t sbase = 0;
        f32x16 acc[8];
        float hin[128];
        __amdgpu_buffer_rsrc_t rs_out = make_rsrc(a.out, 0);
        auto leaves_to = [&](int idx, int tiles) { rs_out = make_rsrc(a.out + (size_t)idx * a.out_stride + (size_t)blk * tiles * 1024, (long long)tiles * 4096); };
        auto leave = [&](auto V) {
            constexpr int v = V;
            __builtin_amdgcn_raw_buffer_store_b32(__builtin_bit_cast(int, hin[v]), rs_out, lane_o, o_value_bytes(v), STORE_NT);
        };
        auto fetch_bits = [&](int idx) {
            const __amdgpu_buffer_rsrc_t rb = make_rsrc(a.bits + (size_t)idx * a.bits_stride + (size_t)blk * 256, 1024);
            return __builtin_bit_cast(u32x4, __builtin_amdgcn_raw_buffer_load_b128(rb, lane16, 0, 0));
        };
        u32x4 bw = fetch_bits(9);
        const float gs = h ? 0.0f : g.w;
        {
            const float b[2] = {h ? g.y : g.x, h ? 0.0f : g.z};
            seg_few<2, 4, true>(acc, ws, sbase, b);
        }
        {
            const int nb = blk + nwaves < n_blocks ? blk + nwaves : blk;
            g = fetch_grad(nb);
        }
        convert_mask<4>(hin, acc, bw);
        bw = fetch_bits(8);
        leaves_to(0, 4);
        seg_hidden<64, 8, true>(acc, ws, sbase, hin, [&](auto S, auto MT) { if constexpr (decltype(MT)::value == 5) leave(S); });
        convert_mask<8>(hin, acc, bw);
        leaves_to(1, 8);
        seg_hidden<128, 8, true>(acc, ws, sbase, hin, [&](auto S, auto MT) { if constexpr (decltype(MT)::value == 5) leave(S); });
        convert_linear<8>(hin, acc);
        static_for<8>([&](auto J) {
            constexpr int j = J;
            bw = fetch_bits(7 - j);
            leaves_to(2 + j, 8);
            seg_hidden<128, 8, true>(acc, ws, sbase, hin, [&](auto S, auto MT) { if constexpr (decltype(MT)::value == 5) leave(S); });
            if constexpr (j == 0) {
                const float b[1] = {gs};
                seg_few<1, 8, false>(acc, ws, sbase, b);
            }
            convert_mask<8>(hin, acc, bw);
        });
        leaves_to(10, 8);
        static_for<128>([&](auto V) { leave(V); });
    }
}

#endif

struct DwWave {
    const float *A; int rtA, a0;
    const float *B; int rtB, b0;
    int shape;
    long long out; int ldc;
    int row0, rows_valid, col0, c_lo, c_hi;
    long long bias_out;
};
struct DwJob { DwWave w[4]; int cost; long long slot_floats, first_float; };
struct DwArgs { const DwJob *jobs; int n_jobs, n_blocks; long long total_cost; float *partial;
                unsigned long long *clocks; };

__host__ __device__ inline long long dw_cut(long long g, long long G, long long W, long long start, long long cost, long long n_blocks) {
    const long long x = g * W / G - start;
    long long b = x <= 0 ? 0 : (x + cost / 2) / cost;
    return b > n_blocks ? n_blocks : b;
}
__host__ __device__ inline long long dw_first_g(long long G, long long W, long long start) { return start * G / W; }
__host__ __device__ inline long long dw_last_g(long long G, long long W, long long start, long long span) { return (start + span - 1) * G / W; }

#ifdef NTX_TRAIN_DW
#ifndef NTX_DW_SYNC
#define NTX_DW_SYNC 16
#endif
constexpr int DW_SYNC = NTX_DW_SYNC;
template <int NA, int NB>
TRN_DEV void dw_piece(const DwWave &tg, float *slot, int blk0, int blk1, int lane) {
    auto uniform_ptr = [](const float *p) {
        const uint32_t lo = (uint32_t)__builtin_amdgcn_readfirstlane((int)(uint32_t)(uintptr_t)p), hi = (uint32_t)__builtin_amdgcn_readfirstlane((int)(uint32_t)((uintptr_t)p >> 32));
        return (const float *)(uintptr_t)(((uint64_t)hi << 32) | (uint64_t)lo);
    };
    const float *A = uniform_ptr(tg.A), *B = uniform_ptr(tg.B);
    const int rtA = __builtin_amdgcn_readfirstlane(tg.rtA), a0 = __builtin_amdgcn_readfirstlane(tg.a0), rtB = __builtin_amdgcn_readfirstlane(tg.rtB), b0 = __builtin_amdgcn_readfirstlane(tg.b0);
    f32x16 acc[NA][NB];
    static_for<NA>([&](auto Ai) { static_for<NB>([&](auto Bi) {
        acc[Ai][Bi] = f32x16{0.f, 0.f, 0.f, 0.f, 0.f, 0.f, 0.f, 0.f, 0.f, 0.f, 0.f, 0.f, 0.f, 0.f, 0.f, 0.f}; }); });
    f32x4 bsum[NB];
    static_for<NB>([&](auto Bi) { bsum[Bi] = f32x4{0.0f, 0.0f, 0.0f, 0.0f}; });
    const bool want_bias = tg.bias_out >= 0;
    const int nblk = blk1 - blk0;
    if (nblk > 0) {
        const __amdgpu_buffer_rsrc_t ra = make_rsrc(A + (size_t)blk0 * rtA * 1024, (long long)nblk * rtA * 4096);
        const __amdgpu_buffer_rsrc_t rb = make_rsrc(B + (size_t)blk0 * rtB * 1024, (long long)nblk * rtB * 4096);
        const uint32_t voff = (uint32_t)lane * 16u;
        const uint32_t stepA = (uint32_t)rtA * 4096u, stepB = (uint32_t)rtB * 4096u, offA = (uint32_t)a0 * 4096u, offB = (uint32_t)b0 * 4096u;
        f32x4 xa[2][NA][2], xb[2][NB][2];
        auto fetch = [&](auto BUF, int i) {
            constexpr int buf = BUF;
#ifdef NTX_X_DWSMALL
            i &= 3;
#endif
#ifdef NTX_X_DWNOLOAD
            if (i > 0) return;
#endif
            const uint32_t oa = (uint32_t)i * stepA + offA + (uint32_t)buf * 2048u, ob = (uint32_t)i * stepB + offB + (uint32_t)buf * 2048u;
            static_for<NA>([&](auto Ai) { static_for<2>([&](auto Q) {
                xa[buf][Ai][Q] = __builtin_bit_cast(f32x4, __builtin_amdgcn_raw_buffer_load_b128(ra, voff, oa + (uint32_t)(decltype(Ai)::value * 4 + decltype(Q)::value) * 1024u, 0)); }); });
            static_for<NB>([&](auto Bi) { static_for<2>([&](auto Q) {
                xb[buf][Bi][Q] = __builtin_bit_cast(f32x4, __builtin_amdgcn_raw_buffer_load_b128(rb, voff, ob + (uint32_t)(decltype(Bi)::value * 4 + decltype(Q)::value) * 1024u, 0)); }); });
        };
        auto compute = [&](auto BUF) {
            constexpr int buf = BUF;
            static_for<2>([&](auto Q) { static_for<4>([&](auto C) {
                constexpr int q = Q, c = C;
                static_for<NA>([&](auto Ai) { static_for<NB>([&](auto Bi) {
                    acc[Ai][Bi] = mfma32(xa[buf][Ai][q][c], xb[buf][Bi][q][c], acc[Ai][Bi]);
                }); });
            }); });
            if (want_bias) static_for<NB>([&](auto Bi) { bsum[Bi] += xb[buf][Bi][0] + xb[buf][Bi][1]; });
        };
        fetch(std::integral_constant<int, 0>{}, 0);
        for (int i = 0; i < nblk; ++i) {
            if ((i & (DW_SYNC - 1)) == 0) __builtin_amdgcn_s_barrier();
            fetch(std::integral_constant<int, 1>{}, i);
            __builtin_amdgcn_sched_barrier(0);
            compute(std::integral_constant<int, 0>{});
            __builtin_amdgcn_sched_barrier(0);
            fetch(std::integral_constant<int, 0>{}, i + 1 < nblk ? i + 1 : i);
            __builtin_amdgcn_sched_barrier(0);
            compute(std::integral_constant<int, 1>{});
            __builtin_amdgcn_sched_barrier(0);
        }
    }
    const int j = lane & 31, hh = lane >> 5;
    const int ldc = __builtin_amdgcn_readfirstlane(tg.ldc), row0 = __builtin_amdgcn_readfirstlane(tg.row0), rows_valid = __builtin_amdgcn_readfirstlane(tg.rows_valid);
    const int col0 = __builtin_amdgcn_readfirstlane(tg.col0), c_lo = __builtin_amdgcn_readfirstlane(tg.c_lo), c_hi = __builtin_amdgcn_readfirstlane(tg.c_hi);
    const long long at_out = (long long)(((uint64_t)(uint32_t)__builtin_amdgcn_readfirstlane((int)(uint32_t)((uint64_t)tg.out >> 32)) << 32) | (uint32_t)__builtin_amdgcn_readfirstlane((int)(uint32_t)(uint64_t)tg.out));
    const __amdgpu_buffer_rsrc_t ro = make_rsrc(slot + at_out, (long long)rows_valid * ldc * 4);
    constexpr uint32_t NOWHERE = 0x7ffffff0u;
    static_for<NB>([&](auto Bi) {
        const int col = col0 + 32 * decltype(Bi)::value + j;
        const bool col_ok = col >= c_lo && col < c_hi;
        const uint32_t coff = (uint32_t)(col - c_lo) * 4u;
        static_for<NA>([&](auto Ai) {
            static_for<16>([&](auto R) {
                constexpr int r = R;
                const int row = row0 + 32 * decltype(Ai)::value + 8 * (r >> 2) + (r & 3) + 4 * hh;
                const uint32_t off = (col_ok && row < rows_valid) ? (uint32_t)(row * ldc) * 4u + coff : NOWHERE;
                __builtin_amdgcn_raw_buffer_store_b32(__builtin_bit_cast(int, (float)acc[Ai][Bi][r]), ro, off, 0, 0);
            });
        });
    });
    if (want_bias) {
        const long long at_bias = (long long)(((uint64_t)(uint32_t)__builtin_amdgcn_readfirstlane((int)(uint32_t)((uint64_t)tg.bias_out >> 32)) << 32) | (uint32_t)__builtin_amdgcn_readfirstlane((int)(uint32_t)(uint64_t)tg.bias_out));
        float *bo = slot + at_bias + (size_t)hh * (c_hi - c_lo);
        static_for<NB>([&](auto Bi) {
            const int col = col0 + 32 * decltype(Bi)::value + j;
            const f32x4 sm = bsum[Bi];
            if (col >= c_lo && col < c_hi) bo[col - c_lo] = (sm.x + sm.y) + (sm.z + sm.w);
        });
    }
}

__global__ __launch_bounds__(256) __attribute__((amdgpu_waves_per_eu(1, 1))) void dw_kernel(DwArgs a) {
    const int lane = threadIdx.x & 63, wave = __builtin_amdgcn_readfirstlane(threadIdx.x >> 6);
    const long long g = blockIdx.x, G = gridDim.x, W = a.total_cost * a.n_blocks;
    long long start = 0;
#ifdef NTX_TRAIN_CLOCKS
    unsigned long long *ck = a.clocks ? a.clocks + (size_t)blockIdx.x * (2 + 3 * a.n_jobs) : nullptr;
    if (ck && threadIdx.x == 0) ck[0] = wall_clock64();
#endif
    for (int jn = 0; jn < a.n_jobs; ++jn) {
        const DwJob &job = a.jobs[jn];
        const long long cost = job.cost, span = cost * a.n_blocks;
        const long long g0 = dw_first_g(G, W, start), g1 = dw_last_g(G, W, start, span);
        if (__builtin_amdgcn_readfirstlane((int)(g >= g0 && g <= g1))) {
            const int blk0 = __builtin_amdgcn_readfirstlane((int)dw_cut(g, G, W, start, cost, a.n_blocks)), blk1 = __builtin_amdgcn_readfirstlane((int)dw_cut(g + 1, G, W, start, cost, a.n_blocks));
            const DwWave &wv = job.w[wave];
            const int shape = __builtin_amdgcn_readfirstlane(wv.shape);
            const int my_slot = __builtin_amdgcn_readfirstlane((int)(g - g0));
            float *slot = a.partial + job.first_float + (long long)my_slot * job.slot_floats;
#ifdef NTX_TRAIN_CLOCKS
            const unsigned long long c0 = wall_clock64();
#endif
            if (shape == 0) dw_piece<4, 4>(wv, slot, blk0, blk1, lane);
            else if (shape == 1) dw_piece<3, 4>(wv, slot, blk0, blk1, lane);
            else if (shape == 2) dw_piece<4, 1>(wv, slot, blk0, blk1, lane);
            else for (int i = 0; i < blk1 - blk0; i += DW_SYNC) __builtin_amdgcn_s_barrier();
#ifdef NTX_TRAIN_CLOCKS
            __syncthreads();
            if (ck && threadIdx.x == 0) { ck[2 + 3 * jn] = (unsigned long long)(blk1 - blk0); ck[3 + 3 * jn] = c0; ck[4 + 3 * jn] = wall_clock64(); }
#endif
        }
        start += span;
    }
#ifdef NTX_TRAIN_CLOCKS
    if (ck && threadIdx.x == 0) ck[1] = wall_clock64();
#endif
}
#endif

constexpr int FWD_VARIANTS[4][2] = {{9, 11}, {9, 8}, {11, 8}, {MAX_PB_GROUPS, MAX_PB_GROUPS}};
void launch_fwd_chain(int variant, bool hoist, hipStream_t st, unsigned grid, const FwdArgs &a);
void launch_dx_chain(hipStream_t st, unsigned grid, const DxArgs &a);
void launch_dw(hipStream_t st, unsigned grid, const DwArgs &a);

}
```

Baseline: 112.5 million ray-samples/s.

## Fold linear feature layer into colour layer weights each step

The feature layer has no activation, so its weights are premultiplied into the first colour layer's position block by a new fold kernel before packing. This removes one 256x256 GEMM layer from both the forward and backward chains and one stored activation and gradient buffer. Weight gradients for the two original layers are recovered afterwards from the folded gradient with two small double-precision fold GEMMs. It also adds an empty asm clobber of a255 to claim the full register file in the chain kernels, and drops debug access to the feature-layer output gradient.

```diff
diff --git a/nerf_tex_amd/csrc/ntx_train.hip b/nerf_tex_amd/csrc/ntx_train.hip
--- a/nerf_tex_amd/csrc/ntx_train.hip
+++ b/nerf_tex_amd/csrc/ntx_train.hip
@@ -229,6 +229,38 @@
     }
     for (int q = 0; z < r.n_split; ++z, ++q) s4[q] += at(z);
     r.out[e] = (s4[0] + s4[1]) + (s4[2] + s4[3]);
+}
+
+struct FoldJob {
+    const float *A; int a_i, a_p;
+    const float *B; int b_p, b_j;
+    const float *a_col, *b_row;
+    const float *a_row, *add;
+    float *C, *C_row;
+};
+struct FoldArgs { FoldJob job[2]; };
+constexpr int FOLD_TILES = 16 * 17;
+__global__ __launch_bounds__(256) void fold_kernel(FoldArgs a) {
+    __shared__ float As[16][17], Bs[16][17];
+    const FoldJob &f = a.job[blockIdx.y];
+    const int ti = blockIdx.x >> 4, tj = blockIdx.x & 15, tx = threadIdx.x & 15, ty = threadIdx.x >> 4;
+    const bool extra = ti == 16;
+    if (extra && !f.a_row) return;
+    const int i = 16 * ti + ty, j = 16 * tj + tx;
+    double acc = 0.0;
+    for (int p0 = 0; p0 < 256; p0 += 16) {
+        As[ty][tx] = extra ? (ty == 0 ? f.a_row[p0 + tx] : 0.0f) : f.A[(size_t)i * f.a_i + (size_t)(p0 + tx) * f.a_p];
+        Bs[ty][tx] = f.B[(size_t)(p0 + ty) * f.b_p + (size_t)j * f.b_j];
+        __syncthreads();
+        for (int q = 0; q < 16; ++q) acc = fma((double)As[ty][q], (double)Bs[q][tx], acc);
+        __syncthreads();
+    }
+    if (extra) {
+        if (ty == 0) f.C_row[j] = (float)(f.add ? acc + (double)f.add[j] : acc);
+    } else {
+        if (f.a_col) acc = fma((double)f.a_col[i], (double)f.b_row[j], acc);
+        f.C[(size_t)i * 256 + j] = (float)acc;
+    }
 }
 
 enum { PACK_HIDDEN = 0, PACK_LINEAR = 1, PACK_AUX_ROW = 2, PACK_AUX_RGB = 3, PACK_COPY = 4 };
@@ -534,6 +566,8 @@
     int Kp = 0, Kd = 0, P = 0, ptiles = 0, dtiles = 0, PS = 0, DS = 0;
     bool ipe = false;
     TLayer trunk[8], feature, c1, c2, rgb, alpha;
+    float *wfold = nullptr;
+    float *fold_m = nullptr;
     size_t n_weights = 0;
     long long cap = 0, cap_blocks = 0, cap_rays = 0;
     float *w = nullptr, *grad = nullptr, *adam_m = nullptr, *adam_v = nullptr;
@@ -565,7 +599,8 @@
     if (!t) return;
     (void)hipSetDevice(t->device);
     void *ptrs[] = {t->w, t->grad, t->adam_m, t->adam_v, t->wfwd, t->wdx, t->aux, t->pack_seg, t->posO, t->dirO, t->sigma, t->raw_rgb, t->z, t->dists, t->noise,
-                    t->dgrad, t->dhead, t->jobs, t->dw_partial, t->stash, t->dirrow, t->color, t->alpha_out, t->ray_loss, t->loss, t->act, t->bits, t->gout};
+                    t->dgrad, t->dhead, t->jobs, t->dw_partial, t->stash, t->dirrow, t->color, t->alpha_out, t->ray_loss, t->loss, t->act, t->bits, t->gout,
+                    t->wfold, t->fold_m};
     for (void *p : ptrs) if (p) (void)hipFree(p);
     delete t;
 }
@@ -653,7 +688,8 @@
     alloc(&t->w, p); alloc(&t->grad, p, true); alloc(&t->adam_m, p, true); alloc(&t->adam_v, p, true);
     alloc(&t->posO, (size_t)NB * t->ptiles * 1024, true); alloc(&t->dirO, (size_t)NB * t->dtiles * 1024, true);
     t->act_stride = t->gout_stride = NB * 8 * 1024; t->bits_stride = NB * 256;
-    alloc(&t->act, (size_t)t->act_stride * 11); alloc((float **)&t->bits, (size_t)t->bits_stride * 10); alloc(&t->gout, (size_t)t->gout_stride * 11);
+    alloc(&t->act, (size_t)t->act_stride * 10); alloc((float **)&t->bits, (size_t)t->bits_stride * 10); alloc(&t->gout, (size_t)t->gout_stride * 10);
+    alloc(&t->wfold, 257 * 256); alloc(&t->fold_m, 256 * 256);
     auto act = [&](int i) { return t->act + (size_t)i * t->act_stride; };
     auto gout = [&](int i) { return t->gout + (size_t)i * t->gout_stride; };
     alloc(&t->sigma, (size_t)M); alloc(&t->raw_rgb, (size_t)M * 3); alloc(&t->z, (size_t)(M + max_rays)); alloc(&t->dists, (size_t)M); alloc(&t->noise, (size_t)M);
@@ -679,15 +715,14 @@
         if (i == 5) { fwd_linear(t->trunk[5], Kp, t->PS); fwd_hidden(t->trunk[5], Kp, 8); }
         else fwd_hidden(t->trunk[i], 0, 8);
     }
-    fwd_hidden(t->feature, 0, 8);
-    fwd_linear(t->c1, Kd, t->DS); fwd_hidden(t->c1, Kd, 8);
+    fwd_linear(t->c1, Kd, t->DS);
+    seg(t->wfold, 256, 1, PACK_HIDDEN, 256, 256, 8, &t->fwd_floats, 128);
     fwd_hidden(t->c2, 0, 4);
     const size_t n_fwd_segs = segs.size();
     auto dx_hidden = [&](const TLayer &l, int row0, int K, int nsteps) { seg(W + l.w + (size_t)row0 * l.out, 1, l.out, PACK_HIDDEN, K, 256, 8, &t->dx_floats, nsteps); };
     seg(W + t->rgb.w, 1, 3, PACK_LINEAR, 3, 128, 4, &t->dx_floats, 2);
     dx_hidden(t->c2, 0, 128, 64);
-    dx_hidden(t->c1, Kd, 256, 128);
-    dx_hidden(t->feature, 0, 256, 128);
+    seg(t->wfold, 1, 256, PACK_HIDDEN, 256, 256, 8, &t->dx_floats, 128);
     seg(W + t->alpha.w, 1, 1, PACK_LINEAR, 1, 256, 8, &t->dx_floats, 1);
     for (int i = 7; i >= 1; --i) dx_hidden(t->trunk[i], i == 5 ? Kp : 0, 256, 128);
     const size_t n_stream_segs = segs.size();
@@ -699,8 +734,7 @@
         first += count; segs.push_back(s);
     };
     for (int i = 0; i < 8; ++i) aux_seg(W + t->trunk[i].b, PACK_AUX_ROW, 256, 256, AUX_BIAS + (size_t)i * 256);
-    aux_seg(W + t->feature.b, PACK_AUX_ROW, 256, 256, AUX_BIAS + 8 * 256); aux_seg(W + t->c1.b, PACK_AUX_ROW, 256, 256, AUX_BIAS + 9 * 256);
-    aux_seg(W + t->c2.b, PACK_AUX_ROW, 128, 256, AUX_BIAS + 10 * 256);
+    aux_seg(t->wfold + 256 * 256, PACK_AUX_ROW, 256, 256, AUX_BIAS + 8 * 256); aux_seg(W + t->c2.b, PACK_AUX_ROW, 128, 256, AUX_BIAS + 9 * 256);
     aux_seg(W + t->alpha.w, PACK_AUX_ROW, 256, 256, AUX_ALPHA_W); aux_seg(W + t->alpha.b, PACK_COPY, 1, 1, AUX_ALPHA_B);
     aux_seg(W + t->rgb.w, PACK_AUX_RGB, 128, 384, AUX_RGB_W); aux_seg(W + t->rgb.b, PACK_COPY, 3, 3, AUX_RGB_B);
     t->pack_total = first; t->n_pack = (int)segs.size();
@@ -716,15 +750,15 @@
             rc = ntx_set_error(NTX_E_HIP, "segment table upload failed");
     }
     std::vector<DwJob> &jobs = t->jobs_host;
-    struct RJ { int job; long long at, count, pair; size_t out; };
+    struct RJ { int job; long long at, count, pair; float *const *base; size_t out; };
     std::vector<RJ> rjobs;
     auto new_job = [&]() { DwJob j{}; for (DwWave &w : j.w) w.shape = -1; jobs.push_back(j); return (int)jobs.size() - 1; };
-    auto matrix = [&](int j, int K, int N, size_t g_kernel, long long g_bias, long long *at_bias) {
+    auto matrix = [&](int j, int K, int N, size_t g_kernel, long long g_bias, long long *at_bias, float *const *kernel_base = nullptr) {
         const long long at = jobs[j].slot_floats;
         jobs[j].slot_floats += (long long)K * N;
-        rjobs.push_back(RJ{j, at, (long long)K * N, 0, g_kernel});
+        rjobs.push_back(RJ{j, at, (long long)K * N, 0, kernel_base ? kernel_base : &t->grad, g_kernel});
         *at_bias = -1;
-        if (g_bias >= 0) { *at_bias = jobs[j].slot_floats; jobs[j].slot_floats += 2 * N; rjobs.push_back(RJ{j, *at_bias, N, N, (size_t)g_bias}); }
+        if (g_bias >= 0) { *at_bias = jobs[j].slot_floats; jobs[j].slot_floats += 2 * N; rjobs.push_back(RJ{j, *at_bias, N, N, &t->grad, (size_t)g_bias}); }
         return at;
     };
     auto wave = [&](int j, int w, int shape, const float *A, int rtA, int a0, const float *B, int rtB, int b0, long long at, int K, int N, int c_lo, long long at_bias) {
@@ -734,29 +768,28 @@
         const int cost = shape == 0 ? 256 : shape == 1 ? 198 : 68;
         if (cost > jobs[j].cost) jobs[j].cost = cost;
     };
-    auto layer_job = [&](const float *X, const float *dY, size_t g_kernel, size_t g_bias) {
-        const int j = new_job(); long long ab; const long long at = matrix(j, 256, 256, g_kernel, (long long)g_bias, &ab);
+    auto layer_job = [&](const float *X, const float *dY, size_t g_kernel, size_t g_bias, float *const *kernel_base = nullptr) {
+        const int j = new_job(); long long ab; const long long at = matrix(j, 256, 256, g_kernel, (long long)g_bias, &ab, kernel_base);
         for (int w = 0; w < 4; ++w) wave(j, w, 0, X, 8, 4 * (w >> 1), dY, 8, 4 * (w & 1), at, 256, 256, 0, ab);
     };
     {
-        const TLayer &r = t->rgb, &al = t->alpha, &c2 = t->c2, &c1 = t->c1, &f = t->feature;
-        for (int i = 7; i >= 1; --i) layer_job(act(i - 1), gout(10 - i), t->trunk[i].w + (size_t)(i == 5 ? Kp : 0) * 256, t->trunk[i].b);
-        layer_job(act(7), gout(2), f.w, f.b);
-        layer_job(act(8), gout(1), c1.w + (size_t)Kd * 256, c1.b);
+        const TLayer &r = t->rgb, &al = t->alpha, &c2 = t->c2, &c1 = t->c1;
+        for (int i = 7; i >= 1; --i) layer_job(act(i - 1), gout(9 - i), t->trunk[i].w + (size_t)(i == 5 ? Kp : 0) * 256, t->trunk[i].b);
+        layer_job(act(7), gout(1), 0, c1.b, &t->fold_m);
         {
             const int j = new_job(); long long ab0, ab5;
             const long long at0 = matrix(j, Kp, 256, t->trunk[0].w, (long long)t->trunk[0].b, &ab0), at5 = matrix(j, Kp, 256, t->trunk[5].w, -1, &ab5);
-            for (int w = 0; w < 2; ++w) { wave(j, w, 1, t->posO, t->ptiles, 0, gout(10), 8, 4 * w, at0, Kp, 256, 0, ab0); wave(j, 2 + w, 1, t->posO, t->ptiles, 0, gout(5), 8, 4 * w, at5, Kp, 256, 0, ab5); }
+            for (int w = 0; w < 2; ++w) { wave(j, w, 1, t->posO, t->ptiles, 0, gout(9), 8, 4 * w, at0, Kp, 256, 0, ab0); wave(j, 2 + w, 1, t->posO, t->ptiles, 0, gout(4), 8, 4 * w, at5, Kp, 256, 0, ab5); }
         }
         {
             const int j = new_job(); long long abd, ab2;
             const long long atd = matrix(j, Kd, 256, c1.w, -1, &abd), at2 = matrix(j, 256, 128, c2.w, (long long)c2.b, &ab2);
-            for (int w = 0; w < 2; ++w) { wave(j, w, 1, t->dirO, t->dtiles, 0, gout(1), 8, 4 * w, atd, Kd, 256, 0, abd); wave(j, 2 + w, 0, act(9), 8, 4 * w, gout(0), 4, 0, at2, 256, 128, 0, ab2); }
+            for (int w = 0; w < 2; ++w) { wave(j, w, 1, t->dirO, t->dtiles, 0, gout(1), 8, 4 * w, atd, Kd, 256, 0, abd); wave(j, 2 + w, 0, act(8), 8, 4 * w, gout(0), 4, 0, at2, 256, 128, 0, ab2); }
         }
         {
             const int j = new_job(); long long abr, aba;
             const long long atr = matrix(j, 128, 3, r.w, (long long)r.b, &abr), ata = matrix(j, 256, 1, al.w, (long long)al.b, &aba);
-            wave(j, 0, 2, act(10), 4, 0, t->dhead, 1, 0, atr, 128, 3, 0, abr);
+            wave(j, 0, 2, act(9), 4, 0, t->dhead, 1, 0, atr, 128, 3, 0, abr);
             for (int w = 0; w < 2; ++w) wave(j, 1 + w, 2, act(7), 8, 4 * w, t->dhead, 1, 0, ata, 256, 1, 3, aba);
         }
     }
@@ -780,7 +813,7 @@
             ReduceJob &r = t->reduce.job[t->reduce.n++];
             const DwJob &j = jobs[rjobs[i].job];
             r.partial = t->dw_partial + j.first_float + rjobs[i].at; r.n_split = 0; r.stride = j.slot_floats; r.count = rjobs[i].count; r.pair = rjobs[i].pair;
-            r.out = t->grad + rjobs[i].out; r.first = rfirst;
+            r.out = *rjobs[i].base + rjobs[i].out; r.first = rfirst;
             rfirst += (rjobs[i].count + 255) / 256 * 256;
             t->reduce_job.push_back(rjobs[i].job);
         }
@@ -816,12 +849,12 @@
     auto act = [&](int i) { return t->act + (size_t)i * t->act_stride; };
     auto gout = [&](int i) { return t->gout + (size_t)i * t->gout_stride; };
     if (layer >= 0 && layer < 8) src = act(layer);
-    else if (layer == 8) src = act(9);
-    else if (layer == 9) { src = act(10); tiles = 4; }
+    else if (layer == 8) src = act(8);
+    else if (layer == 9) { src = act(9); tiles = 4; }
     else if (layer == 10) src = t->sigma;
-    else if (layer >= 20 && layer < 28) src = gout(10 - (layer - 20));
+    else if (layer >= 20 && layer < 28) src = gout(9 - (layer - 20));
     else if (layer == 28) src = gout(1);
-    else if (layer == 29) src = gout(2);
+    else if (layer == 29) return ntx_set_error(NTX_E_UNSUPPORTED, "layer 29: the gradient at the feature layer's output is not kept (the step folds the feature layer into the colour layer)");
     else if (layer == 11) src = t->raw_rgb;
     else if (layer == 30) src = t->dgrad;
     else return ntx_set_error(NTX_E_INVALID, "layer %d (0-7 trunk, 8 / 9 the colour layers, 10 the density, 11 the raw colour; 20-29 the kept gradients, 30 the composite's adjoint)", layer);
@@ -921,7 +954,11 @@
     hipStream_t st = (hipStream_t)stream;
     const long long M = (long long)n_rays * n_samples;
     const int S = n_samples, n_blocks = (int)((M + 31) / 32);
+    const float *Wf = t->w + t->feature.w, *bf = t->w + t->feature.b, *Wc1f = t->w + t->c1.w + (size_t)t->Kd * 256;
     {
+        FoldArgs fa{};
+        fa.job[0] = FoldJob{Wf, 256, 1, Wc1f, 256, 1, nullptr, nullptr, bf, t->w + t->c1.b, t->wfold, t->wfold + 256 * 256};
+        hipLaunchKernelGGL(fold_kernel, dim3(FOLD_TILES, 1), dim3(256), 0, st, fa);
         PackArgs pa{t->pack_seg, t->n_pack, t->pack_total};
         hipLaunchKernelGGL(pack_kernel, dim3((unsigned)((t->pack_total + 255) / 256)), dim3(256), 0, st, pa);
     }
@@ -954,7 +991,7 @@
         const bool hoist = (t->ipe || blur_idx < 0 || blur_idx < t->desc.n_geo) && S % 32 == 0 && getenv("NERFTEX_TRAIN_NO_DIR_HOIST") == nullptr;
         if (hoist) {
             DirRowArgs dr{}; dr.rays_d = rays_d; dr.params = params; dr.rays_per_param_row = rays_per_param_row; dr.n_rays = (int)n_rays; dr.n_geo = t->desc.n_geo;
-            dr.n_app = t->desc.n_app; dr.dir_freq = t->desc.dir_freq; dr.param_freq = t->desc.param_freq; dr.Kd = t->Kd; dr.w = t->w + t->c1.w; dr.bias = t->w + t->c1.b;
+            dr.n_app = t->desc.n_app; dr.dir_freq = t->desc.dir_freq; dr.param_freq = t->desc.param_freq; dr.Kd = t->Kd; dr.w = t->w + t->c1.w; dr.bias = t->wfold + 256 * 256;
             dr.rows = t->dirrow; dr.splice = t->ipe ? blur_idx : -1;
             hipLaunchKernelGGL(dirrow_kernel, dim3((unsigned)n_rays), dim3(256), 0, st, dr);
         }
@@ -1022,6 +1059,14 @@
         const long long total = rb.job[rb.n - 1].first + (rb.job[rb.n - 1].count + 255) / 256 * 256;
         hipLaunchKernelGGL(reduce_batch_kernel, dim3((unsigned)(total / 256)), dim3(256), 0, st, rb);
     }
+    {
+        float *g = t->grad;
+        const float *colsum = g + t->c1.b;
+        FoldArgs fa{};
+        fa.job[0] = FoldJob{Wf, 1, 256, t->fold_m, 256, 1, bf, colsum, nullptr, nullptr, g + t->c1.w + (size_t)t->Kd * 256, nullptr};
+        fa.job[1] = FoldJob{t->fold_m, 256, 1, Wc1f, 1, 256, nullptr, nullptr, colsum, nullptr, g + t->feature.w, g + t->feature.b};
+        hipLaunchKernelGGL(fold_kernel, dim3(FOLD_TILES, 2), dim3(256), 0, st, fa);
+    }
     TRAIN_TRY(hipGetLastError());
     return NTX_OK;
 }
diff --git a/nerf_tex_amd/csrc/ntx_train_device.h b/nerf_tex_amd/csrc/ntx_train_device.h
--- a/nerf_tex_amd/csrc/ntx_train_device.h
+++ b/nerf_tex_amd/csrc/ntx_train_device.h
@@ -27,6 +27,7 @@
 }
 constexpr int STORE_NT = 0;
 constexpr uint32_t o_value_bytes(int V) { return (uint32_t)((V >> 4) * 4096 + ((V & 15) >> 2) * 128 + (V & 3) * 16); }
+TRN_DEV void claim_register_file() { asm volatile("" ::: "a255"); }
 
 template <int R>
 struct WRingT {
@@ -147,10 +148,6 @@
     });
 }
 template <int NMT>
-TRN_DEV void convert_linear(float (&hin)[128], const f32x16 (&prev)[8]) {
-    static_for<NMT * 16>([&](auto V) { constexpr int v = V; hin[v] = prev[v >> 4][v & 15]; });
-}
-template <int NMT>
 TRN_DEV void convert_mask(float (&hin)[128], const f32x16 (&prev)[8], const u32x4 &bits) {
     static_for<NMT * 16>([&](auto V) {
         constexpr int v = V;
@@ -160,7 +157,7 @@
     });
 }
 
-constexpr int AUX_BIAS = 0, AUX_ALPHA_W = 11 * 256, AUX_ALPHA_B = AUX_ALPHA_W + 256, AUX_RGB_W = AUX_ALPHA_B + 4, AUX_RGB_B = AUX_RGB_W + 384,
+constexpr int AUX_BIAS = 0, AUX_ALPHA_W = 10 * 256, AUX_ALPHA_B = AUX_ALPHA_W + 256, AUX_RGB_W = AUX_ALPHA_B + 4, AUX_RGB_B = AUX_RGB_W + 384,
               AUX_FLOATS = AUX_RGB_B + 4;
 template <int MT>
 TRN_DEV void bias_tile(f32x16 (&acc)[8], const float *aux, int layer, int h) {
@@ -187,6 +184,7 @@
 __global__ __launch_bounds__(256) __attribute__((amdgpu_waves_per_eu(1, 1))) void fwd_chain_kernel(FwdArgs a) {
     __shared__ __attribute__((aligned(16))) float aux_lds[AUX_FLOATS];
     __shared__ __attribute__((aligned(16))) float rows_lds[HOIST ? 4 * 256 : 4];
+    claim_register_file();
     ntx::load_aux(aux_lds, a.aux, AUX_FLOATS);
     const int lane = threadIdx.x & 63, n = lane & 31, h = lane >> 5;
     const int wave = __builtin_amdgcn_readfirstlane(blockIdx.x * 4 + (threadIdx.x >> 6)), nwaves = gridDim.x * 4;
@@ -213,7 +211,7 @@
         uint32_t opaque_zero = 0;
         asm volatile("" : "+v"(opaque_zero));
         const float *aux = aux_lds + opaque_zero;
-        const float *rows_aux = rows_lds + opaque_zero + (HOIST ? (threadIdx.x >> 6) * 256 : 0) - AUX_BIAS - 9 * 256;
+        const float *rows_aux = rows_lds + opaque_zero + (HOIST ? (threadIdx.x >> 6) * 256 : 0) - AUX_BIAS - 8 * 256;
         uint32_t sbase = 0;
         f32x16 acc[8];
         float hin[128];
@@ -245,23 +243,20 @@
         auto layer = [&](auto LIc) {
             f32x16 (&cur)[8] = acc; f32x16 (&prev)[8] = acc;
             constexpr int LI = decltype(LIc)::value, in_idx = LI - 1;
-            constexpr bool relu_in = in_idx != 8;
             u32x4 bw = {0u, 0u, 0u, 0u};
-            if constexpr (HOIST && LI == 9) {
+            if constexpr (HOIST && LI == 8) {
                 sbase += (uint32_t)DSG * 8192u;
                 static_for<RING>([&](auto I) { ws.r[I] = wr_load(ws, sbase + (uint32_t)decltype(I)::value * 1024u); });
             }
             static_for<4>([&](auto W) {
                 constexpr int wd = W;
-                if constexpr (relu_in) {
-                    uint32_t w = 0;
-                    static_for<4>([&](auto Q) { convert8_relu_bits<32 * wd + 8 * decltype(Q)::value>(hin, prev, w); });
-                    bw[wd] = w;
-                } else static_for<32>([&](auto V) { constexpr int v = 32 * wd + decltype(V)::value; hin[v] = prev[v >> 4][v & 15]; });
-                const float *bsrc = (HOIST && LI == 9) ? rows_aux : aux;
-                if constexpr (LI < 10 || wd < 2) { bias_tile<2 * wd>(cur, bsrc, LI, h); bias_tile<2 * wd + 1>(cur, bsrc, LI, h); }
+                uint32_t w = 0;
+                static_for<4>([&](auto Q) { convert8_relu_bits<32 * wd + 8 * decltype(Q)::value>(hin, prev, w); });
+                bw[wd] = w;
+                const float *bsrc = (HOIST && LI == 8) ? rows_aux : aux;
+                if constexpr (LI < 9 || wd < 2) { bias_tile<2 * wd>(cur, bsrc, LI, h); bias_tile<2 * wd + 1>(cur, bsrc, LI, h); }
             });
-            if constexpr (relu_in) bits_leave(in_idx < 8 ? in_idx : 8, bw);
+            bits_leave(in_idx, bw);
             if constexpr (LI == 8) {
                 const f32x4 *wa = reinterpret_cast<const f32x4 *>(aux + AUX_ALPHA_W + h * 128);
                 static_for<32>([&](auto I) {
@@ -274,27 +269,27 @@
             __builtin_amdgcn_sched_barrier(0);
             leaves_to(in_idx, 8);
             if constexpr (LI == 5) seg_mem<PSG>(cur, ws, sbase, pb, fetch);
-            if constexpr (LI == 9 && !HOIST) seg_mem<DSG>(cur, ws, sbase, pb, fetch);
+            if constexpr (LI == 8 && !HOIST) seg_mem<DSG>(cur, ws, sbase, pb, fetch);
             if constexpr (LI == 4) rs_in = make_rsrc(a.pos + (size_t)blk * a.ptiles * 1024, (long long)a.ptiles * 4096);
-            if constexpr (LI == 8 && !HOIST) rs_in = make_rsrc(a.dir + (size_t)blk * a.dtiles * 1024, (long long)a.dtiles * 4096);
-            if constexpr (LI == 10) {
+            if constexpr (LI == 7 && !HOIST) rs_in = make_rsrc(a.dir + (size_t)blk * a.dtiles * 1024, (long long)a.dtiles * 4096);
+            if constexpr (LI == 9) {
                 const int nb = blk + nwaves < n_blocks ? blk + nwaves : blk;
                 rs_in = make_rsrc(a.pos + (size_t)nb * a.ptiles * 1024, (long long)a.ptiles * 4096);
             }
             auto extra = [&](auto S, auto MT) {
                 constexpr int s = decltype(S)::value, mt = decltype(MT)::value;
-                if constexpr ((LI == 4 || (LI == 8 && !HOIST) || LI == 10) && mt == 2 && (s == 8 || s == 24)) fetch(std::integral_constant<int, (s == 8 ? 0 : 1)>{});
-                if constexpr (mt == 5 || (LI == 10 && mt == 3)) leave(S);
+                if constexpr ((LI == 4 || (LI == 7 && !HOIST) || LI == 9) && mt == 2 && (s == 8 || s == 24)) fetch(std::integral_constant<int, (s == 8 ? 0 : 1)>{});
+                if constexpr (mt == 5 || (LI == 9 && mt == 3)) leave(S);
             };
-            if constexpr (LI == 10) seg_hidden<128, 4, false>(cur, ws, sbase, hin, extra);
+            if constexpr (LI == 9) seg_hidden<128, 4, false>(cur, ws, sbase, hin, extra);
             else seg_hidden<128, 8, false>(cur, ws, sbase, hin, extra);
         };
-        static_for<10>([&](auto I) { layer(std::integral_constant<int, decltype(I)::value + 1>{}); });
+        static_for<9>([&](auto I) { layer(std::integral_constant<int, decltype(I)::value + 1>{}); });
         {
             u32x4 bw = {0u, 0u, 0u, 0u};
             convert_relu_bits<4>(hin, acc, bw);
             bits_leave(9, bw);
-            leaves_to(10, 4);
+            leaves_to(9, 4);
             static_for<64>([&](auto V) { leave(V); });
             float rgb[3];
             static_for<3>([&](auto C) {
@@ -330,6 +325,7 @@
 
 #ifdef NTX_TRAIN_DX
 __global__ __launch_bounds__(256) __attribute__((amdgpu_waves_per_eu(1, 1))) void dx_chain_kernel(DxArgs a) {
+    claim_register_file();
     const int lane = threadIdx.x & 63, n = lane & 31, h = lane >> 5;
     const int wave = __builtin_amdgcn_readfirstlane(blockIdx.x * 4 + (threadIdx.x >> 6)), nwaves = gridDim.x * 4;
     const int n_blocks = (int)((a.M + 31) >> 5);
@@ -374,13 +370,10 @@
         leaves_to(0, 4);
         seg_hidden<64, 8, true>(acc, ws, sbase, hin, [&](auto S, auto MT) { if constexpr (decltype(MT)::value == 5) leave(S); });
         convert_mask<8>(hin, acc, bw);
-        leaves_to(1, 8);
-        seg_hidden<128, 8, true>(acc, ws, sbase, hin, [&](auto S, auto MT) { if constexpr (decltype(MT)::value == 5) leave(S); });
-        convert_linear<8>(hin, acc);
         static_for<8>([&](auto J) {
             constexpr int j = J;
             bw = fetch_bits(7 - j);
-            leaves_to(2 + j, 8);
+            leaves_to(1 + j, 8);
             seg_hidden<128, 8, true>(acc, ws, sbase, hin, [&](auto S, auto MT) { if constexpr (decltype(MT)::value == 5) leave(S); });
             if constexpr (j == 0) {
                 const float b[1] = {gs};
@@ -388,7 +381,7 @@
             }
             convert_mask<8>(hin, acc, bw);
         });
-        leaves_to(10, 8);
+        leaves_to(9, 8);
         static_for<128>([&](auto V) { leave(V); });
     }
 }
```

Result: no change. 112.5 million ray-samples/s (median of 3 runs) (-0.0%).
